# alenzhao/Mitty

Hardware: AMD Instinct MI355X
Metric: paired 2x150bp reads/sec at 30x WGS, 1/2/4/8 MI355X; qname POS/CIGAR bit-exact (higher is better)
Workload: dtype int64+u8

## Files before the change

### include/mitty_hip.h

```cpp
#ifndef MITTY_HIP_H
#define MITTY_HIP_H

#include <stdint.h>

#ifdef __cplusplus
extern "C" {
#endif

typedef struct mh_ctx mh_ctx;

enum {
  MH_OK = 0,
  MH_E_ARG = -1,
  MH_E_HIP = -2,
  MH_E_OOM = -3,
  MH_E_CAPACITY = -4,
  MH_E_COMPLEX_VARIANT = -5,
  MH_E_SEED = -6,
  MH_E_STATE = -7,
  MH_E_NO_DEVICE = -8
};

enum { MH_RNG_MITTY = 0, MH_RNG_PHILOX = 1 };

int32_t mh_version(void);
int32_t mh_device_count(int32_t *out);
int32_t mh_create(int32_t device, mh_ctx **out);
int32_t mh_destroy(mh_ctx *ctx);
const char *mh_last_error(const mh_ctx *ctx);
int32_t mh_sync(mh_ctx *ctx);

int32_t mh_selftest_scan_fault(mh_ctx *ctx);
int32_t mh_selftest_scan(mh_ctx *ctx, int32_t kind, int32_t fields, const int64_t *in, int64_t n, int32_t repeat,
                         int64_t *incl, int64_t *excl, int64_t *total, int64_t *info);
int32_t mh_selftest_sort(mh_ctx *ctx, const uint32_t *keys, int64_t n, int32_t end_bit, uint32_t *keys_out,
                         uint32_t *vals_out);

int32_t mh_read_model_params(int64_t mean_rlen, double coverage, double *p, int64_t *passes);
int32_t mh_work_units(uint64_t seed, const int32_t *ploidy, int64_t n_regions, int64_t passes,
                      int32_t *out_region, int32_t *out_cpy, uint32_t *out_seed, int64_t *out_n);

int32_t mh_upload_contig(mh_ctx *ctx, int32_t contig_id, const char *seq, int64_t len);
int32_t mh_release_contig(mh_ctx *ctx, int32_t contig_id);
int32_t mh_build_haplotype(mh_ctx *ctx, int32_t slot, int32_t contig_id, int64_t ref_start_pos,
                           const int64_t *v_pos, const uint8_t *v_op, const int64_t *v_oplen,
                           const int64_t *v_alt_off, const int64_t *v_alt_len, const char *alt_pool,
                           int64_t alt_pool_len, int64_t n_var,
                           int64_t *out_n_nodes, int64_t *out_p_min, int64_t *out_p_max);
int32_t mh_upload_variants(mh_ctx *ctx, int32_t vset, const int64_t *v_pos, const uint8_t *v_op,
                           const int64_t *v_oplen, const int64_t *v_alt_off, const int64_t *v_alt_len,
                           const char *alt_pool, int64_t alt_pool_len, int64_t n_var);
int32_t mh_build_haplotype_vset(mh_ctx *ctx, int32_t slot, int32_t contig_id, int64_t ref_start_pos, int32_t vset,
                                int64_t *out_n_nodes, int64_t *out_p_min, int64_t *out_p_max);
int32_t mh_build_haplotypes_vset(mh_ctx *ctx, int32_t n, const int32_t *slots, const int32_t *contig_ids,
                                 const int64_t *ref_starts, const int32_t *vsets, int64_t *out_n_nodes,
                                 int64_t *out_p_min, int64_t *out_p_max);
int32_t mh_prefetch_haplotypes_vset(mh_ctx *ctx, int32_t n, const int32_t *slots, const int32_t *contig_ids,
                                    const int64_t *ref_starts, const int32_t *vsets, int32_t n_units,
                                    const int32_t *unit_slots, const uint64_t *unit_seeds, double p);
int32_t mh_release_variants(mh_ctx *ctx, int32_t vset);
int32_t mh_get_nodes(mh_ctx *ctx, int32_t slot, int64_t *ps, int64_t *pr, uint8_t *op, int64_t *oplen,
                     char *hap, int64_t hap_cap, int64_t *hap_len);
int32_t mh_get_haplotype_aux(mh_ctx *ctx, int32_t slot, char *rc, int64_t rc_cap, int64_t *hap_len,
                             int64_t *run_start, int64_t *run_end, int64_t run_cap, int64_t *n_runs,
                             int32_t *bkt, int64_t bkt_cap, int64_t *n_bkt);
int32_t mh_release_haplotype(mh_ctx *ctx, int32_t slot);
int32_t mh_expand_variant(int64_t samp_pos, int64_t ref_pos, int64_t ref_start_pos, int64_t v_pos, int32_t op,
                          int64_t oplen, int64_t *out, int32_t *n_nodes, int64_t *samp_next, int64_t *ref_next);

int32_t mh_sample_templates(mh_ctx *ctx, int32_t slot, double p, int32_t rlen, const double *cum_tlen,
                            int32_t n_tlen, uint64_t seed, int32_t rng_mode, int64_t *out_n_templates);
int32_t mh_sample_templates_span(mh_ctx *ctx, int64_t p_min, int64_t p_max, double p, int32_t rlen,
                                 const double *cum_tlen, int32_t n_tlen, uint64_t seed, int32_t rng_mode,
                                 int64_t *out_n_templates);
int32_t mh_sample_units(mh_ctx *ctx, int32_t n_units, const int32_t *tpl_ids, const int32_t *slots,
                        const uint64_t *seeds, double p, int32_t rlen, const double *cum_tlen, int32_t n_tlen,
                        int32_t rng_mode, int64_t *out_n);
int32_t mh_sample_units_async(mh_ctx *ctx, int32_t n_units, const int32_t *tpl_ids, const int32_t *slots,
                              const uint64_t *seeds, double p, int32_t rlen, const double *cum_tlen, int32_t n_tlen,
                              int32_t rng_mode);
int32_t mh_templates_count(mh_ctx *ctx, int32_t tpl_id, int64_t *n);
int32_t mh_use_templates(mh_ctx *ctx, int32_t tpl_id);
int32_t mh_release_templates(mh_ctx *ctx, int32_t tpl_id);
int32_t mh_set_templates(mh_ctx *ctx, const int8_t *fo0, const int64_t *pos0, const int64_t *pos1, int64_t n,
                         int32_t rlen);
int32_t mh_get_templates(mh_ctx *ctx, int8_t *fo0, int64_t *pos0, int64_t *pos1, int64_t cap, int64_t *n);
int32_t mh_templates_export(mh_ctx *ctx, int32_t tpl_id, int32_t on_device, int8_t *fo0, int64_t *pos0,
                            int64_t *pos1, int64_t cap, int64_t *n);
int32_t mh_templates_import(mh_ctx *ctx, int32_t tpl_id, int32_t on_device, const int8_t *fo0, const int64_t *pos0,
                            const int64_t *pos1, int64_t n, int32_t rlen);
#define MH_GC_BINS 101
int32_t mh_gc_thin(mh_ctx *ctx, int32_t tpl_id, int32_t slot, const uint64_t *accept , uint64_t seed,
                   uint64_t unit_key, int64_t *out_n, int64_t *bin_seen ,
                   int64_t *bin_kept );

int32_t mh_emit_reads(mh_ctx *ctx, int32_t slot, const char *serial_stub, const char *chrom, int64_t cpy,
                      int32_t write_fastq2, uint64_t unit_key, int64_t *out_kept, int64_t *out_bytes1,
                      int64_t *out_bytes2);
int32_t mh_emit_prepare(mh_ctx *ctx, int32_t slot, const char *serial_stub, const char *chrom, int64_t cpy,
                        int32_t write_fastq2, uint64_t unit_key, int64_t *out_kept, int64_t *out_b1, int64_t *out_b2);
int32_t mh_emit_reads_range(mh_ctx *ctx, int32_t slot, const char *serial_stub, const char *chrom, int64_t cpy,
                            int32_t write_fastq2, uint64_t unit_key, int64_t t_begin, int64_t t_end,
                            int64_t cnt_base, int64_t *out_kept, int64_t *out_bytes1, int64_t *out_bytes2);
int32_t mh_emit_reads_async(mh_ctx *ctx, int32_t slot, const char *serial_stub, const char *chrom, int64_t cpy,
                            int32_t write_fastq2, uint64_t unit_key);
int32_t mh_emit_collect(mh_ctx *ctx, int64_t *out, int64_t cap, int64_t *n_units);
int32_t mh_emit_measure(mh_ctx *ctx, int32_t slot, const char *serial_stub, const char *chrom, int64_t cpy,
                        int32_t write_fastq2, uint64_t unit_key, int64_t t_begin, int64_t t_end, int64_t cnt_base,
                        int64_t *out_kept, int64_t *out_b1, int64_t *out_b2);
int32_t mh_count_kept(mh_ctx *ctx, int32_t slot, int64_t t_begin, int64_t t_end, int64_t *out_kept);
int32_t mh_output_size(mh_ctx *ctx, int64_t *bytes1, int64_t *bytes2);
int32_t mh_output_fetch(mh_ctx *ctx, int64_t offset1, char *fq1, int64_t len1, int64_t offset2, char *fq2,
                        int64_t len2);
int32_t mh_output_fetch_async(mh_ctx *ctx, int64_t offset1, char *fq1, int64_t len1, int64_t offset2, char *fq2,
                              int64_t len2, int32_t *ticket);
int32_t mh_output_fetch_wait(mh_ctx *ctx, int32_t ticket);
int32_t mh_output_reset(mh_ctx *ctx);
int32_t mh_host_alloc(int64_t bytes, void **out);
int32_t mh_host_free(void *p);
// ... 52 lines not shown
int32_t mh_score_add_store(mh_ctx *ctx);
int32_t mh_score_result(mh_ctx *ctx, uint64_t *mq_mat, uint64_t *derr_mat, int64_t *counts);
int32_t mh_score_reset(mh_ctx *ctx);

#define MH_MODEL_NO_RLEN INT64_MAX
int32_t mh_model_begin(mh_ctx *ctx, int32_t n_refs, int32_t every, int32_t min_mq, int32_t max_bq, int32_t max_bp,
                       int32_t max_tlen);
int32_t mh_model_add_records(mh_ctx *ctx, const uint8_t *recs, int64_t len, const int64_t *roff, int64_t n);
int32_t mh_model_add_store(mh_ctx *ctx);
int32_t mh_model_result(mh_ctx *ctx, uint64_t *bq_mat, uint64_t *tlen_mat, int64_t *counts);
int32_t mh_model_reset(mh_ctx *ctx);

#define MH_COV_NO_POS INT64_MAX
int32_t mh_cov_begin(mh_ctx *ctx, int32_t n_refs, const int64_t *lengths, int64_t block_len);
int32_t mh_cov_add_records(mh_ctx *ctx, const uint8_t *recs, int64_t len, const int64_t *roff, int64_t n);
int32_t mh_cov_add_store(mh_ctx *ctx);
int32_t mh_cov_gc(mh_ctx *ctx, int32_t ref_index, int32_t contig_id);
int32_t mh_cov_result(mh_ctx *ctx, int32_t ref_index, uint32_t *n_n, uint32_t *n_gc, int64_t *covered,
                      uint64_t *span_sum, int64_t *min_pos, int64_t *max_end, int64_t n_blocks, int64_t *counts);
int32_t mh_cov_reset(mh_ctx *ctx);

#define MH_BQ_MAX_BP 500
#define MH_BQ_MAX_BQ 100
int32_t mh_bq_begin(mh_ctx *ctx, int32_t n_refs);
int32_t mh_bq_add_records(mh_ctx *ctx, const uint8_t *recs, int64_t len, const int64_t *roff, int64_t n);
int32_t mh_bq_add_store(mh_ctx *ctx);
int32_t mh_bq_result(mh_ctx *ctx, int32_t ref_index, uint64_t *mat, int64_t *counts);
int32_t mh_bq_reset(mh_ctx *ctx);

typedef struct mh_vcf mh_vcf;
int32_t mh_vcf_open(const char *path, const char *sample, mh_vcf **out);
const char *mh_vcf_error(const mh_vcf *v);
int32_t mh_vcf_close(mh_vcf *v);
int32_t mh_vcf_region(mh_vcf *v, const char *chrom, int64_t start0, int64_t end, int32_t *ploidy, int64_t *n_var,
                      int64_t *alt_bytes, int32_t cap);
int32_t mh_vcf_copy(mh_vcf *v, int32_t cpy, int64_t *pos, uint8_t *op, int64_t *oplen, int64_t *alt_off,
                    int64_t *alt_len, char *alt_pool);
int32_t mh_vcf_filter(const char *in_path, const char *sample, int32_t n_regions, const char *chroms,
                      const int64_t *start0, const int64_t *end, const char *out_path, int32_t bgzf, int32_t threads,
                      int64_t *n_written, int64_t *n_filtered, char *err, int32_t err_cap);

typedef struct mh_fasta mh_fasta;
int32_t mh_fasta_open(const char *path, const char *names, mh_fasta **out);
const char *mh_fasta_error(const mh_fasta *f);
int32_t mh_fasta_count(const mh_fasta *f, int32_t *n);
int32_t mh_fasta_contig(const mh_fasta *f, int32_t i, const char **name, const char **seq, int64_t *len);
int32_t mh_fasta_copy(const mh_fasta *f, int32_t i, char *dst);
int32_t mh_fasta_close(mh_fasta *f);

int32_t mh_bgzf_compress(const char *in, int64_t len, int32_t level, int32_t threads, char *out, int64_t cap,
                         int64_t *used);
int32_t mh_bgzf_eof(char *out28);
int32_t mh_bgzf_compress_device(mh_ctx *ctx, const void *d_in, int64_t len, void *d_out, int64_t cap,
                                int64_t *used);
int32_t mh_bgzf_compress_gpu(mh_ctx *ctx, const char *in, int64_t len, char *out, int64_t cap, int64_t *used);
int32_t mh_bgzf_inflate_gpu(int32_t device, const char *in, int64_t len, char *out, int64_t cap, int64_t *used,
                            int64_t *bad_offset);
int32_t mh_output_bgzf(mh_ctx *ctx, int32_t file, char *out, int64_t cap, int64_t *used);
int32_t mh_selftest_bgzf(mh_ctx *ctx, const char *in, int64_t len, int32_t misalign, char *out, int64_t cap,
                         int64_t *used);
int32_t mh_output_bgzf_range(mh_ctx *ctx, int32_t file, int64_t offset, int64_t len, char *out, int64_t cap,
                             int64_t *used);
int32_t mh_output_bgzf_pair(mh_ctx *ctx, int64_t offset, int64_t n1, int64_t n2, char *out1, int64_t cap1,
                            char *out2, int64_t cap2, int64_t *used1, int64_t *used2, int32_t *ticket);
int32_t mh_output_bgzf_wait(mh_ctx *ctx, int32_t ticket);

int32_t mh_corrupt_fastq(mh_ctx *ctx, const char *fq1, int64_t len1, const char *fq2, int64_t len2, int64_t t_base,
                         int64_t *used1, int64_t *used2, int64_t *templates);

int32_t mh_set_corruption(mh_ctx *ctx, int32_t enable, const double *cum_bq, int32_t max_bp, int32_t n_bq,
                          const double *phred_p, uint64_t seed);
int32_t mh_set_corruption_stream(mh_ctx *ctx, int32_t rng_mode, uint64_t seed, const uint32_t *key624, int32_t pos);
int32_t mh_get_corruption_stream(mh_ctx *ctx, uint32_t *key624, int32_t *pos, int64_t *words);

int32_t mh_stage_times(mh_ctx *ctx, const char **names, double *ms, int32_t cap, int32_t *n);
int32_t mh_enable_timing(mh_ctx *ctx, int32_t on);

int32_t mh_mt_window_at(uint32_t seed, uint64_t offset, uint32_t *out624);
int32_t mh_set_emit_mode(mh_ctx *ctx, int32_t mode);
#define MH_DEC_SEQUENTIAL 1
#define MH_DEC_FORCE_FIXUP 2
#define MH_DEC_FORCE_GEO 4
int32_t mh_set_decode_mode(mh_ctx *ctx, int32_t mode);
int32_t mh_fixup_count(mh_ctx *ctx, int64_t *n);

#ifdef __cplusplus
}
#endif
#endif
```

### mitty_amd/_native.py

```python
import ctypes
import os
import sys

import numpy as np

LIB_PATH = (os.environ.get('MH_LIB') or
            os.path.join(os.path.dirname(os.path.abspath(__file__)), '_lib', 'libmitty_hip.so'))

MH_OK, MH_E_ARG, MH_E_HIP, MH_E_OOM, MH_E_CAPACITY, MH_E_COMPLEX_VARIANT, MH_E_SEED, MH_E_STATE, MH_E_NO_DEVICE = \
  0, -1, -2, -3, -4, -5, -6, -7, -8
MH_RNG_MITTY, MH_RNG_PHILOX = 0, 1

EXPORTS = ['mh_version', 'mh_device_count', 'mh_create', 'mh_destroy', 'mh_last_error', 'mh_sync',
           'mh_selftest_scan_fault', 'mh_selftest_scan', 'mh_selftest_sort', 'mh_selftest_bgzf',
           'mh_read_model_params', 'mh_work_units', 'mh_upload_contig', 'mh_release_contig', 'mh_build_haplotype', 'mh_upload_variants', 'mh_build_haplotype_vset', 'mh_build_haplotypes_vset', 'mh_prefetch_haplotypes_vset', 'mh_release_variants', 'mh_get_nodes', 'mh_get_haplotype_aux',
           'mh_release_haplotype', 'mh_expand_variant', 'mh_sample_templates', 'mh_sample_templates_span', 'mh_set_templates',
           'mh_get_templates', 'mh_templates_export', 'mh_templates_import', 'mh_gc_thin', 'mh_emit_reads', 'mh_emit_prepare', 'mh_emit_reads_async', 'mh_emit_collect', 'mh_output_size', 'mh_output_fetch', 'mh_output_reset', 'mh_host_alloc', 'mh_host_free', 'mh_device_cache_trim', 'mh_device_live_bytes',
           'mh_read_batch', 'mh_set_corruption', 'mh_set_corruption_stream', 'mh_get_corruption_stream', 'mh_stage_times', 'mh_enable_timing', 'mh_sample_units', 'mh_sample_units_async', 'mh_templates_count',
           'mh_use_templates', 'mh_release_templates', 'mh_mt_window_at', 'mh_fixup_count', 'mh_set_emit_mode', 'mh_set_decode_mode',
           'mh_emit_reads_range', 'mh_emit_measure', 'mh_count_kept', 'mh_bam_set_refs', 'mh_bam_add_fastq', 'mh_bam_add_output',
           'mh_bam_records', 'mh_bam_set_capacity', 'mh_bam_set_spill_dir', 'mh_bam_spilled', 'mh_bam_export', 'mh_bam_import', 'mh_bam_sort', 'mh_bam_write', 'mh_bam_write_gpu', 'mh_bam_reset', 'mh_bam_partition', 'mh_bam_partition_fetch', 'mh_bam_import_tie', 'mh_bam_sorted_head', 'mh_bam_write_part', 'mh_bam_bai_runs', 'mh_corrupt_fastq', 'mh_bgzf_compress', 'mh_bgzf_eof', 'mh_bgzf_compress_device', 'mh_bgzf_compress_gpu', 'mh_output_bgzf',
           'mh_output_bgzf_range', 'mh_output_bgzf_pair', 'mh_output_bgzf_wait', 'mh_output_fetch_async',
           'mh_output_fetch_wait',
           'mh_vcf_open', 'mh_vcf_error', 'mh_vcf_close', 'mh_vcf_region', 'mh_vcf_copy', 'mh_vcf_filter',
           'mh_bamfile_open', 'mh_bamfile_open_gpu', 'mh_bgzf_inflate_gpu', 'mh_bamfile_error', 'mh_bamfile_header', 'mh_bamfile_next', 'mh_bamfile_close',
           'mh_score_begin', 'mh_score_add_records', 'mh_score_add_store', 'mh_score_result', 'mh_score_reset',
           'mh_model_begin', 'mh_model_add_records', 'mh_model_add_store', 'mh_model_result', 'mh_model_reset',
           'mh_cov_begin', 'mh_cov_add_records', 'mh_cov_add_store', 'mh_cov_gc', 'mh_cov_result', 'mh_cov_reset',
           'mh_bq_begin', 'mh_bq_add_records', 'mh_bq_add_store', 'mh_bq_result', 'mh_bq_reset',
           'mh_fasta_open', 'mh_fasta_error', 'mh_fasta_count', 'mh_fasta_contig', 'mh_fasta_copy', 'mh_fasta_close']


MODEL_NO_RLEN = (1 << 63) - 1
GC_BINS = 101
MASK64 = (1 << 64) - 1
COV_NO_POS = (1 << 63) - 1
BQ_MAX_BP, BQ_MAX_BQ = 500, 100


class NativeError(RuntimeError):
  pass


class NativeUnavailable(NativeError):
  pass


_lib = None

c_i32, c_i64, c_u64, c_dbl, c_vp = ctypes.c_int32, ctypes.c_int64, ctypes.c_uint64, ctypes.c_double, ctypes.c_void_p
P_i64 = ctypes.POINTER(c_i64)


def _sig(L, name, args, res=c_i32):
  f = getattr(L, name)
  f.argtypes = args
  f.restype = res


def lib():
  global _lib
  if _lib is not None:
    return _lib
  if not os.path.exists(LIB_PATH):
    raise NativeUnavailable('libmitty_hip.so not built ({}); run __graft_entry__.build() or make -C '
                            'mitty_amd/csrc'.format(LIB_PATH))
  if 'torch' not in sys.modules and int(os.environ.get('WORLD_SIZE', '1')) > 1:
    import torch
  L = ctypes.CDLL(LIB_PATH)
  _sig(L, 'mh_version', [])
  _sig(L, 'mh_device_count', [ctypes.POINTER(c_i32)])
  _sig(L, 'mh_create', [c_i32, ctypes.POINTER(c_vp)])
  _sig(L, 'mh_destroy', [c_vp])
  _sig(L, 'mh_last_error', [c_vp], ctypes.c_char_p)
  _sig(L, 'mh_sync', [c_vp])
  _sig(L, 'mh_selftest_scan_fault', [c_vp])
  _sig(L, 'mh_selftest_scan', [c_vp, c_i32, c_i32, c_vp, c_i64, c_i32, c_vp, c_vp, c_vp, c_vp])
  _sig(L, 'mh_selftest_sort', [c_vp, c_vp, c_i64, c_i32, c_vp, c_vp])
  _sig(L, 'mh_selftest_bgzf', [c_vp, c_vp, c_i64, c_i32, c_vp, c_i64, P_i64])
  _sig(L, 'mh_read_model_params', [c_i64, c_dbl, ctypes.POINTER(c_dbl), P_i64])
  _sig(L, 'mh_work_units', [c_u64, c_vp, c_i64, c_i64, c_vp, c_vp, c_vp, P_i64])
  _sig(L, 'mh_upload_contig', [c_vp, c_i32, c_vp, c_i64])
  _sig(L, 'mh_release_contig', [c_vp, c_i32])
  _sig(L, 'mh_upload_variants', [c_vp, c_i32, c_vp, c_vp, c_vp, c_vp, c_vp, c_vp, c_i64, c_i64])
  _sig(L, 'mh_build_haplotype_vset', [c_vp, c_i32, c_i32, c_i64, c_i32, c_vp, c_vp, c_vp])
  _sig(L, 'mh_release_variants', [c_vp, c_i32])
  _sig(L, 'mh_build_haplotype', [c_vp, c_i32, c_i32, c_i64, c_vp, c_vp, c_vp, c_vp, c_vp, c_vp, c_i64, c_i64,
                                 P_i64, P_i64, P_i64])
  _sig(L, 'mh_get_nodes', [c_vp, c_i32, c_vp, c_vp, c_vp, c_vp, c_vp, c_i64, P_i64])
  _sig(L, 'mh_get_haplotype_aux', [c_vp, c_i32, c_vp, c_i64, P_i64, c_vp, c_vp, c_i64, P_i64, c_vp, c_i64, P_i64])
  _sig(L, 'mh_release_haplotype', [c_vp, c_i32])
  _sig(L, 'mh_bgzf_compress_device', [c_vp, c_vp, c_i64, c_vp, c_i64, P_i64])
  _sig(L, 'mh_bgzf_compress_gpu', [c_vp, c_vp, c_i64, c_vp, c_i64, P_i64])
  _sig(L, 'mh_output_bgzf', [c_vp, c_i32, c_vp, c_i64, P_i64])
  _sig(L, 'mh_output_bgzf_range', [c_vp, c_i32, c_i64, c_i64, c_vp, c_i64, P_i64])
  _sig(L, 'mh_output_bgzf_pair', [c_vp, c_i64, c_i64, c_i64, c_vp, c_i64, c_vp, c_i64, P_i64, P_i64,
                                  ctypes.POINTER(c_i32)])
  _sig(L, 'mh_output_bgzf_wait', [c_vp, c_i32])
  _sig(L, 'mh_output_fetch_async', [c_vp, c_i64, c_vp, c_i64, c_i64, c_vp, c_i64, ctypes.POINTER(c_i32)])
  _sig(L, 'mh_output_fetch_wait', [c_vp, c_i32])
  _sig(L, 'mh_expand_variant', [c_i64, c_i64, c_i64, c_i64, c_i32, c_i64, P_i64, ctypes.POINTER(c_i32), P_i64, P_i64])
  _sig(L, 'mh_sample_templates', [c_vp, c_i32, c_dbl, c_i32, c_vp, c_i32, c_u64, c_i32, P_i64])
  _sig(L, 'mh_sample_templates_span', [c_vp, c_i64, c_i64, c_dbl, c_i32, c_vp, c_i32, c_u64, c_i32, P_i64])
  _sig(L, 'mh_set_templates', [c_vp, c_vp, c_vp, c_vp, c_i64, c_i32])
  _sig(L, 'mh_get_templates', [c_vp, c_vp, c_vp, c_vp, c_i64, P_i64])
  _sig(L, 'mh_emit_reads', [c_vp, c_i32, ctypes.c_char_p, ctypes.c_char_p, c_i64, c_i32, c_u64, P_i64, P_i64, P_i64])
  _sig(L, 'mh_emit_prepare', [c_vp, c_i32, ctypes.c_char_p, ctypes.c_char_p, c_i64, c_i32, c_u64, P_i64, P_i64, P_i64])
  _sig(L, 'mh_emit_reads_async', [c_vp, c_i32, ctypes.c_char_p, ctypes.c_char_p, c_i64, c_i32, c_u64])
  _sig(L, 'mh_emit_collect', [c_vp, c_vp, c_i64, P_i64])
  _sig(L, 'mh_build_haplotypes_vset', [c_vp, c_i32, c_vp, c_vp, c_vp, c_vp, c_vp, c_vp, c_vp])
  _sig(L, 'mh_prefetch_haplotypes_vset', [c_vp, c_i32, c_vp, c_vp, c_vp, c_vp, c_i32, c_vp, c_vp, c_dbl])
  _sig(L, 'mh_emit_reads_range', [c_vp, c_i32, ctypes.c_char_p, ctypes.c_char_p, c_i64, c_i32, c_u64, c_i64, c_i64,
                                   c_i64, P_i64, P_i64, P_i64])
  _sig(L, 'mh_count_kept', [c_vp, c_i32, c_i64, c_i64, P_i64])
  _sig(L, 'mh_emit_measure', [c_vp, c_i32, ctypes.c_char_p, ctypes.c_char_p, c_i64, c_i32, c_u64, c_i64, c_i64, c_i64,
                              P_i64, P_i64, P_i64])
  _sig(L, 'mh_bam_set_refs', [c_vp, c_i32, ctypes.c_char_p, c_vp])
  _sig(L, 'mh_bam_add_fastq', [c_vp, c_vp, c_i64, c_vp, c_i64, c_i64, P_i64, P_i64, P_i64])
  _sig(L, 'mh_bam_add_output', [c_vp, c_i64, P_i64])
  _sig(L, 'mh_bam_records', [c_vp, P_i64, P_i64])
  _sig(L, 'mh_bam_set_capacity', [c_vp, c_i64])
  _sig(L, 'mh_bam_spilled', [c_vp, P_i64, P_i64])
  _sig(L, 'mh_bam_export', [c_vp, c_i64, c_i64, c_vp, c_vp, c_vp, c_vp])
  _sig(L, 'mh_bam_import', [c_vp, c_vp, c_vp, c_vp, c_vp, c_i64])
  _sig(L, 'mh_bam_partition', [c_vp, c_vp, c_i32, ctypes.c_uint64, c_vp, c_vp, c_vp])
  _sig(L, 'mh_bam_set_spill_dir', [c_vp, ctypes.c_char_p])
  _sig(L, 'mh_bam_partition_fetch', [c_vp, c_vp, c_i64])
  _sig(L, 'mh_bam_import_tie', [c_vp, c_vp, c_vp, c_vp, c_vp, c_vp, c_i64])
  _sig(L, 'mh_bam_sorted_head', [c_vp, c_i64, c_vp])
  _sig(L, 'mh_bam_write_part', [c_vp, ctypes.c_char_p, ctypes.c_char_p, c_i64, c_i64, c_vp, c_i64, c_i32, P_i64,
                                P_i64, P_i64, c_vp, c_i64])
  _sig(L, 'mh_bam_bai_runs', [c_vp, P_i64, c_vp, c_i64, P_i64, c_vp, c_i64, c_vp])
  _sig(L, 'mh_bam_write', [c_vp, ctypes.c_char_p, ctypes.c_char_p, c_i64, c_i32, c_i32, ctypes.c_char_p, P_i64,
                           P_i64])
  _sig(L, 'mh_bam_write_gpu', [c_vp, ctypes.c_char_p, ctypes.c_char_p, c_i64, ctypes.c_char_p, P_i64, P_i64, P_i64])
  _sig(L, 'mh_bam_reset', [c_vp])
  _sig(L, 'mh_bam_sort', [c_vp])
  _sig(L, 'mh_corrupt_fastq', [c_vp, c_vp, c_i64, c_vp, c_i64, c_i64, P_i64, P_i64, P_i64])
  _sig(L, 'mh_bgzf_compress', [c_vp, c_i64, c_i32, c_i32, c_vp, c_i64, P_i64])
  _sig(L, 'mh_bgzf_eof', [c_vp])
  _sig(L, 'mh_vcf_open', [ctypes.c_char_p, ctypes.c_char_p, ctypes.POINTER(c_vp)])
  _sig(L, 'mh_vcf_error', [c_vp], ctypes.c_char_p)
  _sig(L, 'mh_vcf_close', [c_vp])
  _sig(L, 'mh_vcf_region', [c_vp, ctypes.c_char_p, c_i64, c_i64, ctypes.POINTER(c_i32), c_vp, c_vp, c_i32])
  _sig(L, 'mh_vcf_copy', [c_vp, c_i32, c_vp, c_vp, c_vp, c_vp, c_vp, c_vp])
  _sig(L, 'mh_vcf_filter', [ctypes.c_char_p, ctypes.c_char_p, c_i32, c_vp, c_vp, c_vp, ctypes.c_char_p, c_i32, c_i32,
                            P_i64, P_i64, ctypes.c_char_p, c_i32])
  _sig(L, 'mh_bamfile_open', [ctypes.c_char_p, c_i32, ctypes.POINTER(c_vp)])
  _sig(L, 'mh_bamfile_open_gpu', [ctypes.c_char_p, c_i32, c_i32, ctypes.POINTER(c_vp)])
  _sig(L, 'mh_bgzf_inflate_gpu', [c_i32, c_vp, c_i64, c_vp, c_i64, P_i64, P_i64])
  _sig(L, 'mh_bamfile_error', [c_vp], ctypes.c_char_p)
  _sig(L, 'mh_bamfile_header', [c_vp, ctypes.POINTER(c_vp), P_i64, ctypes.POINTER(c_i32), ctypes.POINTER(c_vp),
                                ctypes.POINTER(c_vp)])
  _sig(L, 'mh_bamfile_next', [c_vp, c_i64, ctypes.POINTER(c_vp), P_i64, ctypes.POINTER(c_vp), P_i64])
  _sig(L, 'mh_bamfile_close', [c_vp])
  _sig(L, 'mh_score_begin', [c_vp, c_i32, ctypes.c_char_p, c_i32, c_i32, c_i32, ctypes.c_char_p])
  _sig(L, 'mh_score_add_records', [c_vp, c_vp, c_i64, c_vp, c_i64])
  _sig(L, 'mh_score_add_store', [c_vp])
  _sig(L, 'mh_score_result', [c_vp, c_vp, c_vp, c_vp])
  _sig(L, 'mh_score_reset', [c_vp])
  _sig(L, 'mh_model_begin', [c_vp, c_i32, c_i32, c_i32, c_i32, c_i32, c_i32])
  _sig(L, 'mh_model_add_records', [c_vp, c_vp, c_i64, c_vp, c_i64])
  _sig(L, 'mh_model_add_store', [c_vp])
  _sig(L, 'mh_model_result', [c_vp, c_vp, c_vp, c_vp])
  _sig(L, 'mh_model_reset', [c_vp])
  _sig(L, 'mh_cov_begin', [c_vp, c_i32, c_vp, c_i64])
  _sig(L, 'mh_cov_add_records', [c_vp, c_vp, c_i64, c_vp, c_i64])
  _sig(L, 'mh_cov_add_store', [c_vp])
  _sig(L, 'mh_cov_gc', [c_vp, c_i32, c_i32])
  _sig(L, 'mh_cov_result', [c_vp, c_i32, c_vp, c_vp, c_vp, c_vp, c_vp, c_vp, c_i64, c_vp])
  _sig(L, 'mh_cov_reset', [c_vp])
  _sig(L, 'mh_bq_begin', [c_vp, c_i32])
  _sig(L, 'mh_bq_add_records', [c_vp, c_vp, c_i64, c_vp, c_i64])
  _sig(L, 'mh_bq_add_store', [c_vp])
  _sig(L, 'mh_bq_result', [c_vp, c_i32, c_vp, c_vp])
  _sig(L, 'mh_bq_reset', [c_vp])
  _sig(L, 'mh_fasta_open', [ctypes.c_char_p, c_vp, ctypes.POINTER(c_vp)])
  _sig(L, 'mh_fasta_error', [c_vp], ctypes.c_char_p)
  _sig(L, 'mh_fasta_count', [c_vp, ctypes.POINTER(c_i32)])
  _sig(L, 'mh_fasta_contig', [c_vp, c_i32, ctypes.POINTER(ctypes.c_char_p), ctypes.POINTER(c_vp), P_i64])
  _sig(L, 'mh_fasta_copy', [c_vp, c_i32, c_vp])
  _sig(L, 'mh_fasta_close', [c_vp])
  _sig(L, 'mh_output_size', [c_vp, P_i64, P_i64])
  _sig(L, 'mh_output_fetch', [c_vp, c_i64, c_vp, c_i64, c_i64, c_vp, c_i64])
  _sig(L, 'mh_output_reset', [c_vp])
  _sig(L, 'mh_host_alloc', [c_i64, ctypes.POINTER(c_vp)])
  _sig(L, 'mh_host_free', [c_vp])
  _sig(L, 'mh_device_cache_trim', [ctypes.POINTER(c_i64)])
  _sig(L, 'mh_device_live_bytes', [ctypes.POINTER(c_i64), ctypes.POINTER(c_i64), c_i32])
  _sig(L, 'mh_read_batch', [c_vp, c_i32, c_vp, c_vp, c_i64, c_vp, c_vp, c_vp,
                            c_vp, c_i64, c_vp, P_i64, c_vp, c_i64, c_vp, P_i64, c_vp, c_i64, c_vp, P_i64])
  _sig(L, 'mh_set_corruption', [c_vp, c_i32, c_vp, c_i32, c_i32, c_vp, c_u64])
  _sig(L, 'mh_templates_export', [c_vp, c_i32, c_i32, c_vp, c_vp, c_vp, c_i64, P_i64])
  _sig(L, 'mh_templates_import', [c_vp, c_i32, c_i32, c_vp, c_vp, c_vp, c_i64, c_i32])
  _sig(L, 'mh_gc_thin', [c_vp, c_i32, c_i32, c_vp, c_u64, c_u64, P_i64, c_vp, c_vp])
  _sig(L, 'mh_set_corruption_stream', [c_vp, c_i32, c_u64, c_vp, c_i32])
  _sig(L, 'mh_get_corruption_stream', [c_vp, c_vp, ctypes.POINTER(c_i32), P_i64])
  _sig(L, 'mh_stage_times', [c_vp, ctypes.POINTER(ctypes.c_char_p), ctypes.POINTER(c_dbl), c_i32,
                             ctypes.POINTER(c_i32)])
  _sig(L, 'mh_enable_timing', [c_vp, c_i32])
  _sig(L, 'mh_sample_units', [c_vp, c_i32, c_vp, c_vp, c_vp, c_dbl, c_i32, c_vp, c_i32, c_i32, c_vp])
  _sig(L, 'mh_sample_units_async', [c_vp, c_i32, c_vp, c_vp, c_vp, c_dbl, c_i32, c_vp, c_i32, c_i32])
  _sig(L, 'mh_templates_count', [c_vp, c_i32, c_vp])
  _sig(L, 'mh_use_templates', [c_vp, c_i32])
  _sig(L, 'mh_release_templates', [c_vp, c_i32])
  _sig(L, 'mh_mt_window_at', [ctypes.c_uint32, c_u64, c_vp])
  _sig(L, 'mh_fixup_count', [c_vp, P_i64])
  _sig(L, 'mh_set_emit_mode', [c_vp, c_i32])
  _sig(L, 'mh_set_decode_mode', [c_vp, c_i32])
  _lib = L
  return L


def mt_window_at(seed, offset):
  out = np.empty(624, np.uint32)
  rc = lib().mh_mt_window_at(int(seed), int(offset), _ptr(out))
  if rc:
    _raise(rc, 'mh_mt_window_at failed')
  return out


def bgzf_compress(data, level=6, threads=8):
  n = len(data)
  src = np.frombuffer(data, np.uint8) if n else np.zeros(1, np.uint8)
  cap = n + (n // 0xff00 + 1) * 64 + 64
  out = np.empty(cap, np.uint8)
  used = c_i64()
  rc = lib().mh_bgzf_compress(_ptr(src), n, int(level), int(threads), _ptr(out), cap, ctypes.byref(used))
  if rc == MH_E_CAPACITY:
    out = np.empty(used.value, np.uint8)
    rc = lib().mh_bgzf_compress(_ptr(src), n, int(level), int(threads), _ptr(out), used.value, ctypes.byref(used))
  if rc:
    _raise(rc, 'mh_bgzf_compress failed')
  return out[:used.value].tobytes()


class VcfFile:

  def __init__(self, path, sample):
    L = lib()
    self._L = L
    self._h = c_vp()
    rc = L.mh_vcf_open(path.encode(), sample.encode(), ctypes.byref(self._h))
    if rc:
      msg = L.mh_vcf_error(self._h).decode() if self._h else 'mh_vcf_open failed'
      self.close()
      _raise(rc, msg)

  def close(self):
    if getattr(self, '_h', None):
      self._L.mh_vcf_close(self._h)
      self._h = None

  def __del__(self):
    try:
      self.close()
    except Exception:
      pass

  def region(self, chrom, start0, end):
    pl = c_i32()
    nv = np.zeros(64, np.int64)
    ab = np.zeros(64, np.int64)
    rc = self._L.mh_vcf_region(self._h, chrom.encode(), int(start0), int(end), ctypes.byref(pl), _ptr(nv), _ptr(ab),
                               64)
    if rc:
      _raise(rc, self._L.mh_vcf_error(self._h).decode())
    copies = []
    for c in range(pl.value):
      n, nb = int(nv[c]), int(ab[c])
      pos, oplen, aoff, alen = (np.empty(n, np.int64) for _ in range(4))
      op = np.empty(n, np.uint8)
      pool = np.empty(max(nb, 1), np.uint8)
      rc = self._L.mh_vcf_copy(self._h, c, _ptr(pos), _ptr(op), _ptr(oplen), _ptr(aoff), _ptr(alen), _ptr(pool))
      if rc:
        _raise(rc, self._L.mh_vcf_error(self._h).decode())
      copies.append({'pos': pos, 'op': op, 'oplen': oplen, 'alt_off': aoff, 'alt_len': alen,
                     'alt_pool': pool[:nb].tobytes()})
    return pl.value, copies


class BamFile:

  def __init__(self, path, threads=2, device=None):
    L = lib()
    self._L = L
    self._h = c_vp()
    if device is None:
      rc = L.mh_bamfile_open(path.encode(), int(threads), ctypes.byref(self._h))
    else:
      rc = L.mh_bamfile_open_gpu(path.encode(), int(device), int(threads), ctypes.byref(self._h))
    if rc:
# ... 294 lines not shown
    us, ud = a(unit_slots, np.int32), a(unit_seeds, np.uint64)
    self._chk(self._L.mh_prefetch_haplotypes_vset(self._h, n, _ptr(s), _ptr(c), _ptr(r), _ptr(v), nu, _ptr(us),
                                                  _ptr(ud), float(p)))

  def release_variants(self, vset):
    self._chk(self._L.mh_release_variants(self._h, int(vset)))

  def get_nodes(self, slot, n_nodes, with_hap=True):
    ps, pr, ol = (np.empty(max(n_nodes, 1), np.int64) for _ in range(3))
    op = np.empty(max(n_nodes, 1), np.uint8)
    hl = c_i64()
    self._chk(self._L.mh_get_nodes(self._h, slot, None, None, None, None, None, 0, ctypes.byref(hl)))
    hap = np.empty(max(hl.value, 1), np.uint8) if with_hap else None
    self._chk(self._L.mh_get_nodes(self._h, slot, _ptr(ps), _ptr(pr), _ptr(op), _ptr(ol), _ptr(hap),
                                   hl.value if with_hap else 0, ctypes.byref(hl)))
    return ps[:n_nodes], pr[:n_nodes], op[:n_nodes], ol[:n_nodes], (hap[:hl.value].tobytes() if with_hap else None)

  def get_haplotype_aux(self, slot):
    hl, nr, nb = c_i64(), c_i64(), c_i64()
    self._chk(self._L.mh_get_haplotype_aux(self._h, slot, None, 0, ctypes.byref(hl), None, None, 0, ctypes.byref(nr),
                                           None, 0, ctypes.byref(nb)))
    rc = np.empty(max(hl.value, 1), np.uint8)
    rs, re_ = np.empty(max(nr.value, 1), np.int64), np.empty(max(nr.value, 1), np.int64)
    bkt = np.empty(nb.value + 1, np.int32)
    self._chk(self._L.mh_get_haplotype_aux(self._h, slot, _ptr(rc), hl.value, ctypes.byref(hl), _ptr(rs), _ptr(re_),
                                           nr.value, ctypes.byref(nr), _ptr(bkt), nb.value + 1, ctypes.byref(nb)))
    return rc[:hl.value].tobytes(), rs[:nr.value], re_[:nr.value], bkt

  def release_haplotype(self, slot):
    self._chk(self._L.mh_release_haplotype(self._h, slot))

  def sample_templates(self, slot, p, rlen, cum_tlen, seed, rng_mode=MH_RNG_MITTY):
    ct = np.ascontiguousarray(cum_tlen, dtype=np.float64)
    n = c_i64()
    self._chk(self._L.mh_sample_templates(self._h, slot, float(p), int(rlen), _ptr(ct), len(ct), int(seed),
                                          int(rng_mode), ctypes.byref(n)))
    return n.value

  def sample_templates_span(self, p_min, p_max, p, rlen, cum_tlen, seed, rng_mode=MH_RNG_MITTY):
    if not (0 <= int(seed) <= 0xffffffff):
      raise ValueError('Seed value {} is out of range 0 - {}'.format(seed, 0xffffffff))
    ct = np.ascontiguousarray(cum_tlen, dtype=np.float64)
    n = c_i64()
    self._chk(self._L.mh_sample_templates_span(self._h, int(p_min), int(p_max), float(p), int(rlen), _ptr(ct),
                                               len(ct), int(seed), int(rng_mode), ctypes.byref(n)))
    return n.value

  def sample_units(self, tpl_ids, slots, seeds, p, rlen, cum_tlen, rng_mode=MH_RNG_MITTY):
    ids = np.ascontiguousarray(tpl_ids, dtype=np.int32)
    sl = np.ascontiguousarray(slots, dtype=np.int32)
    sd = np.ascontiguousarray(seeds, dtype=np.uint64)
    ct = np.ascontiguousarray(cum_tlen, dtype=np.float64)
    out = np.zeros(max(len(ids), 1), dtype=np.int64)
    self._chk(self._L.mh_sample_units(self._h, len(ids), _ptr(ids), _ptr(sl), _ptr(sd), float(p), int(rlen),
                                      _ptr(ct), len(ct), int(rng_mode), _ptr(out)))
    return out[:len(ids)]

  def sample_units_async(self, tpl_ids, slots, seeds, p, rlen, cum_tlen, rng_mode=MH_RNG_MITTY):
    ids = np.ascontiguousarray(tpl_ids, dtype=np.int32)
    sl = np.ascontiguousarray(slots, dtype=np.int32)
    sd = np.ascontiguousarray(seeds, dtype=np.uint64)
    ct = np.ascontiguousarray(cum_tlen, dtype=np.float64)
    self._chk(self._L.mh_sample_units_async(self._h, len(ids), _ptr(ids), _ptr(sl), _ptr(sd), float(p), int(rlen),
                                            _ptr(ct), len(ct), int(rng_mode)))
    return len(ids)

  def template_count(self, tpl_id):
    n = c_i64()
    self._chk(self._L.mh_templates_count(self._h, int(tpl_id), ctypes.byref(n)))
    return n.value

  def use_templates(self, tpl_id):
    self._chk(self._L.mh_use_templates(self._h, int(tpl_id)))

  def release_templates(self, tpl_id):
    self._chk(self._L.mh_release_templates(self._h, int(tpl_id)))

  def set_emit_mode(self, mode):
    self._chk(self._L.mh_set_emit_mode(self._h, int(mode)))

  def set_decode_mode(self, mode):
    self._chk(self._L.mh_set_decode_mode(self._h, int(mode)))

  def fixup_count(self):
    n = c_i64()
    self._chk(self._L.mh_fixup_count(self._h, ctypes.byref(n)))
    return n.value

  def set_templates(self, fo0, pos0, pos1, rlen):
    fo0 = np.ascontiguousarray(fo0, dtype=np.int8)
    pos0 = np.ascontiguousarray(pos0, dtype=np.int64)
    pos1 = np.ascontiguousarray(pos1, dtype=np.int64)
    self._chk(self._L.mh_set_templates(self._h, _ptr(fo0), _ptr(pos0), _ptr(pos1), len(fo0), int(rlen)))

  def get_templates(self):
    n = c_i64()
    self._L.mh_get_templates(self._h, None, None, None, 0, ctypes.byref(n))
    m = n.value
    fo0, p0, p1 = np.empty(max(m, 1), np.int8), np.empty(max(m, 1), np.int64), np.empty(max(m, 1), np.int64)
    self._chk(self._L.mh_get_templates(self._h, _ptr(fo0), _ptr(p0), _ptr(p1), max(m, 1), ctypes.byref(n)))
    return fo0[:m], p0[:m], p1[:m]

  def emit_prepare(self, slot, serial_stub, chrom, cpy, write_fastq2=True, unit_key=0, wait=True):
    if not wait:
      self._chk(self._L.mh_emit_prepare(self._h, slot, serial_stub.encode(), chrom.encode(), int(cpy),
                                        1 if write_fastq2 else 0, int(unit_key), None, None, None))
      return None
    k, b1, b2 = c_i64(), c_i64(), c_i64()
    self._chk(self._L.mh_emit_prepare(self._h, slot, serial_stub.encode(), chrom.encode(), int(cpy),
                                      1 if write_fastq2 else 0, int(unit_key), ctypes.byref(k), ctypes.byref(b1),
                                      ctypes.byref(b2)))
    return k.value, b1.value, b2.value

  def emit_reads(self, slot, serial_stub, chrom, cpy, write_fastq2=True, unit_key=0, t_range=None, cnt_base=0):
    k, b1, b2 = c_i64(), c_i64(), c_i64()
    if t_range is None:
      self._chk(self._L.mh_emit_reads(self._h, slot, serial_stub.encode(), chrom.encode(), int(cpy),
                                      1 if write_fastq2 else 0, int(unit_key), ctypes.byref(k), ctypes.byref(b1),
                                      ctypes.byref(b2)))
    else:
      self._chk(self._L.mh_emit_reads_range(self._h, slot, serial_stub.encode(), chrom.encode(), int(cpy),
                                            1 if write_fastq2 else 0, int(unit_key), int(t_range[0]),
                                            int(t_range[1]), int(cnt_base), ctypes.byref(k), ctypes.byref(b1),
                                            ctypes.byref(b2)))
    return k.value, b1.value, b2.value

  def emit_async(self, slot, serial_stub, chrom, cpy, write_fastq2=True, unit_key=0):
    self._chk(self._L.mh_emit_reads_async(self._h, slot, serial_stub.encode(), chrom.encode(), int(cpy),
                                          1 if write_fastq2 else 0, int(unit_key)))

  def emit_collect(self):
    n = c_i64()
    self._chk(self._L.mh_emit_collect(self._h, None, 0, ctypes.byref(n)))
    out = np.zeros(3 * max(n.value, 1), np.int64)
    self._chk(self._L.mh_emit_collect(self._h, _ptr(out), n.value, ctypes.byref(n)))
    return [tuple(int(x) for x in out[3 * i:3 * i + 3]) for i in range(n.value)]

  def emit_measure(self, slot, serial_stub, chrom, cpy, write_fastq2=True, unit_key=0, t_range=None, cnt_base=0):
    k, b1, b2 = c_i64(), c_i64(), c_i64()
    t0, t1 = t_range if t_range is not None else (0, -1)
    self._chk(self._L.mh_emit_measure(self._h, slot, serial_stub.encode(), chrom.encode(), int(cpy),
                                      1 if write_fastq2 else 0, int(unit_key), int(t0), int(t1), int(cnt_base),
                                      ctypes.byref(k), ctypes.byref(b1), ctypes.byref(b2)))
    return k.value, b1.value, (b2.value if write_fastq2 else 0)

  def bgzf_range(self, f, off, n, pin):
    if n <= 0:
      return b''
    cap = n + (n // 0xff00 + 2) * 40 + 64
    pin.reserve(cap)
    used = c_i64()
    self._chk(self._L.mh_output_bgzf_range(self._h, int(f), int(off), int(n), c_vp(pin.ptr), cap, ctypes.byref(used)))
    return bytes(pin.view(used.value))

  def count_kept(self, slot, t_begin, t_end):
    k = c_i64()
    self._chk(self._L.mh_count_kept(self._h, slot, int(t_begin), int(t_end), ctypes.byref(k)))
    return k.value

  def output_size(self):
    a, b = c_i64(), c_i64()
    self._chk(self._L.mh_output_size(self._h, ctypes.byref(a), ctypes.byref(b)))
    return a.value, b.value

  def fetch_output(self, off1=0, len1=None, off2=0, len2=None):
    u1, u2 = self.output_size()
# ... 355 lines not shown
    caps = [max(64, 64 * n), max(64, 16 * n), max(64, int(l.sum()) + 16 if n else 64)]
    for _ in range(2):
      bufs = [np.empty(c, np.uint8) for c in caps]
      rc = self._L.mh_read_batch(self._h, slot, _ptr(p), _ptr(l), n, _ptr(pos), _ptr(n0), _ptr(n1),
                                 _ptr(bufs[0]), caps[0], _ptr(offs[0]), ctypes.byref(used[0]),
                                 _ptr(bufs[1]), caps[1], _ptr(offs[1]), ctypes.byref(used[1]),
                                 _ptr(bufs[2]), caps[2], _ptr(offs[2]), ctypes.byref(used[2]))
      if rc == MH_E_CAPACITY:
        caps = [max(c, u.value + 16) for c, u in zip(caps, used)]
        continue
      self._chk(rc)
      break
    texts = [b[:u.value].tobytes().decode('latin-1') for b, u in zip(bufs, used)]
    return pos[:n], n0[:n], n1[:n], texts, offs

  def set_corruption(self, enable, cum_bq=None, phred_p=None, seed=0):
    if not enable:
      self._chk(self._L.mh_set_corruption(self._h, 0, None, 0, 0, None, 0))
      return
    cb = np.ascontiguousarray(cum_bq, dtype=np.float64)
    ph = np.ascontiguousarray(phred_p, dtype=np.float64)
    self._chk(self._L.mh_set_corruption(self._h, 1, _ptr(cb), cb.shape[1], cb.shape[2], _ptr(ph), int(seed)))

  def templates_export(self, tpl_id, fo0=None, pos0=None, pos1=None, cap=None):
    n = c_i64()
    if fo0 is not None:
      self._chk(self._L.mh_templates_export(self._h, int(tpl_id), 1, c_vp(fo0), c_vp(pos0), c_vp(pos1), int(cap),
                                            ctypes.byref(n)))
      return n.value
    self._L.mh_templates_export(self._h, int(tpl_id), 0, None, None, None, 0, ctypes.byref(n))
    m = n.value
    a, b, c = np.empty(max(m, 1), np.int8), np.empty(max(m, 1), np.int64), np.empty(max(m, 1), np.int64)
    self._chk(self._L.mh_templates_export(self._h, int(tpl_id), 0, _ptr(a), _ptr(b), _ptr(c), max(m, 1),
                                          ctypes.byref(n)))
    return a[:m], b[:m], c[:m]

  def templates_import(self, tpl_id, n, rlen, fo0, pos0, pos1, on_device=False):
    if on_device:
      self._chk(self._L.mh_templates_import(self._h, int(tpl_id), 1, c_vp(fo0), c_vp(pos0), c_vp(pos1), int(n),
                                            int(rlen)))
      return
    a = np.ascontiguousarray(fo0, dtype=np.int8)
    b = np.ascontiguousarray(pos0, dtype=np.int64)
    c = np.ascontiguousarray(pos1, dtype=np.int64)
    self._chk(self._L.mh_templates_import(self._h, int(tpl_id), 0, _ptr(a), _ptr(b), _ptr(c), int(n), int(rlen)))

  def gc_thin(self, tpl_id, slot, accept, seed, unit_key):
    acc = np.ascontiguousarray(accept, dtype=np.uint64)
    if acc.shape != (GC_BINS,):
      raise ValueError('gc_thin: {} thresholds needed, got an array of shape {}'.format(GC_BINS, acc.shape))
    n = c_i64()
    seen, kept = np.zeros(GC_BINS, np.int64), np.zeros(GC_BINS, np.int64)
    self._chk(self._L.mh_gc_thin(self._h, int(tpl_id), int(slot), _ptr(acc), int(seed) & MASK64, int(unit_key) & MASK64,
                                 ctypes.byref(n), _ptr(seen), _ptr(kept)))
    return n.value, seen, kept

  def set_corruption_stream(self, rng_mode, seed=0, key=None, pos=624):
    k = None if key is None else np.ascontiguousarray(key, dtype=np.uint32)
    if k is not None and k.shape != (624,):
      raise ValueError('MT19937 key must hold 624 words')
    self._chk(self._L.mh_set_corruption_stream(self._h, int(rng_mode), int(seed), None if k is None else _ptr(k),
                                               int(pos)))

  def get_corruption_stream(self):
    key = np.empty(624, np.uint32)
    pos, words = c_i32(), c_i64()
    self._chk(self._L.mh_get_corruption_stream(self._h, _ptr(key), ctypes.byref(pos), ctypes.byref(words)))
    return key, pos.value, words.value

  def enable_timing(self, on=True):
    self._chk(self._L.mh_enable_timing(self._h, 1 if on else 0))

  def stage_times(self):
    n = c_i32()
    self._L.mh_stage_times(self._h, None, None, 0, ctypes.byref(n))
    names = (ctypes.c_char_p * max(n.value, 1))()
    ms = (c_dbl * max(n.value, 1))()
    self._L.mh_stage_times(self._h, names, ms, n.value, ctypes.byref(n))
    return [(names[i].decode(), ms[i]) for i in range(n.value)]

  def sync(self):
    self._chk(self._L.mh_sync(self._h))

  def selftest_sort(self, keys, end_bit):
    import numpy as np
    k = np.ascontiguousarray(keys, dtype=np.uint32)
    ko, vo = np.empty_like(k), np.empty_like(k)
    self._chk(self._L.mh_selftest_sort(self._h, k.ctypes.data, k.size, int(end_bit), ko.ctypes.data, vo.ctypes.data))
    return ko, vo

  def selftest_scan(self, kind, x, repeat=1):
    x = np.ascontiguousarray(x, dtype=np.int64)
    if x.ndim not in (1, 2):
      raise ValueError('selftest_scan: a 1-d or 2-d array')
    fields = 1 if x.ndim == 1 else x.shape[1]
    n = x.shape[0]
    scans = int(kind) != 3
    incl = np.empty_like(x) if scans else None
    excl = np.empty_like(x) if scans else None
    total, info = np.zeros(max(fields, 1), np.int64), np.zeros(2, np.int64)
    self._chk(self._L.mh_selftest_scan(self._h, int(kind), int(fields), _ptr(x), n, int(repeat), _ptr(incl),
                                       _ptr(excl), _ptr(total), _ptr(info)))
    return incl, excl, (total[0] if x.ndim == 1 else total), (int(info[0]), int(info[1]))

  def selftest_bgzf(self, data, misalign=0):
    n = len(data)
    if n == 0:
      return b''
    src = np.frombuffer(data, np.uint8)
    out = np.empty(n + (n // 0xff00 + 2) * 40 + 64, np.uint8)
    used = c_i64()
    self._chk(self._L.mh_selftest_bgzf(self._h, _ptr(src), n, int(misalign), _ptr(out), len(out), ctypes.byref(used)))
    return out[:used.value].tobytes()

  def selftest_scan_fault(self):
    rc = self._L.mh_selftest_scan_fault(self._h)
    return rc, self._L.mh_last_error(self._h).decode(errors='replace')


def expand_variant(samp_pos, ref_pos, ref_start_pos, v_pos, op, oplen):
  out = (c_i64 * 10)()
  n, sn, rn = c_i32(), c_i64(), c_i64()
  rc = lib().mh_expand_variant(int(samp_pos), int(ref_pos), int(ref_start_pos), int(v_pos), ord(op), int(oplen), out,
                               ctypes.byref(n), ctypes.byref(sn), ctypes.byref(rn))
  if rc:
    _raise(rc, 'mh_expand_variant: bad variant (op {!r}, oplen {})'.format(op, oplen))
  return [(out[5 * j], out[5 * j + 1], chr(out[5 * j + 2]), out[5 * j + 3], out[5 * j + 4])
          for j in range(n.value)], sn.value, rn.value
```

### mitty_amd/csrc/mh_api.hip

```cpp
#include <sys/mman.h>
#include <sys/syscall.h>
#include <unistd.h>

#include <algorithm>
#include <atomic>
#include <cctype>
#include <cstdio>
#include <unordered_map>
#include <chrono>
#include <cmath>
#include <condition_variable>
#include <cstring>
#include <map>
#include <mutex>
#include <thread>
#include <type_traits>

#include "mh_bgzf.h"
#include <vector>

#include "mh_corrupt.h"
#include "mh_internal.h"
#include "mh_scan.h"
#include "mh_sort.h"
// ... 422 lines not shown
      hipEventCreateWithFlags(&ctx->ev_ready, hipEventDisableTiming) != hipSuccess ||
      hipEventCreateWithFlags(&ctx->ev_writer, hipEventDisableTiming) != hipSuccess ||
      [&] {
        for (auto &e : ctx->eset)
          if (hipEventCreateWithFlags(&e.done, hipEventDisableTiming) != hipSuccess ||
              hipEventCreateWithFlags(&e.rb, hipEventDisableTiming) != hipSuccess ||
              hipHostMalloc((void **)&e.h_stat, 64 + 8192, hipHostMallocDefault) != hipSuccess)
            return true;
        return false;
      }()) {
    delete ctx;
    return MH_E_HIP;
  }
  hipDeviceProp_t prop;
  if (hipGetDeviceProperties(&prop, device) == hipSuccess) ctx->max_cu = prop.multiProcessorCount;
  *out = ctx;
  return MH_OK;
}

int32_t mh_destroy(mh_ctx *ctx) {
  if (!ctx) return MH_OK;
  if (ctx->pf_thread.joinable()) ctx->pf_thread.join();
  (void)hipSetDevice(ctx->device);
  (void)hipStreamSynchronize(ctx->wstream);
  (void)hipStreamSynchronize(ctx->stream);
  if (ctx->stream2) (void)hipStreamSynchronize(ctx->stream2);
  if (ctx->pstream) (void)hipStreamSynchronize(ctx->pstream);
  for (auto x : ctx->xstream)
    if (x) (void)hipStreamSynchronize(x);
  for (auto &kv : ctx->contigs) release(kv.second.seq);
  for (auto &kv : ctx->haps) release_hap(kv.second);
  for (auto &h : ctx->hap_spare) release_hap(h);
  for (auto &kv : ctx->vsets) release_vars(kv.second);
  for (auto &kv : ctx->tsets) {
    release(kv.second.fo0); release(kv.second.pos0); release(kv.second.pos1); release(kv.second.n0);
    if (kv.second.used) (void)hipEventDestroy(kv.second.used);
  }
  release(ctx->jump_polys); release(ctx->perm_tmp); release(ctx->nrun_tmp); release(ctx->dec_buf);
  release(ctx->gc_buf);
  for (auto &b : ctx->gc_out) release(b);
  for (auto &b : ctx->pb) release(b);
  release(ctx->pb_tmp);
  release(ctx->gz_slots); release(ctx->gz_tok); release(ctx->gz_info); release(ctx->gz_off); release(ctx->gz_scan); release(ctx->gz_out);
  release(ctx->gz_in);
  for (auto &b : ctx->s) release(b);
  for (auto &b : ctx->lane2) release(b);
  for (auto &l : ctx->xlane)
    for (auto &b : l) release(b);
  for (auto &b : ctx->xscan) release(b);
  release(ctx->scan_partials); release(ctx->scan_partials2); release(ctx->d_small);
  release(ctx->corrupt_cum); release(ctx->corrupt_phred);
  release(ctx->out1); release(ctx->out2);
  release(ctx->cr_rows);
  release(ctx->cr_codes);
  release(ctx->scan_partials_w);
  for (auto &b : ctx->sl2) release(b);
  for (auto &b : ctx->sl3) release(b);
  ctx->tail_state.reset();
  for (hipEvent_t e : ctx->ev_gz)
    if (e) (void)hipEventDestroy(e);
  for (hipEvent_t e : ctx->ev_fetch)
    if (e) (void)hipEventDestroy(e);
  if (ctx->h_small) (void)hipHostFree(ctx->h_small);
  if (ctx->h_small3) (void)hipHostFree(ctx->h_small3);
  if (ctx->h_units) (void)hipHostFree(ctx->h_units);
  for (uint8_t *p : ctx->h_bam_pin)
    if (p) (void)hipHostFree(p);
  for (auto &e : ctx->eset) {
    release(e.recs); release(e.off); release(e.tsum); release(e.tpre); release(e.stat); release(e.crrec);
    (void)hipEventDestroy(e.done);
    if (e.rb) (void)hipEventDestroy(e.rb);
    if (e.h_stat) (void)hipHostFree(e.h_stat);
  }
  (void)hipEventDestroy(ctx->ev_ready);
  (void)hipEventDestroy(ctx->ev_writer);
  (void)hipStreamDestroy(ctx->wstream);
  bam_release(ctx->bam);
  score_release(ctx->score);
  model_release(ctx->model);
  model_release(ctx->bq);
  cov_release(ctx->cov);
  if (ctx->ev_fork) (void)hipEventDestroy(ctx->ev_fork);
  if (ctx->ev_join) (void)hipEventDestroy(ctx->ev_join);
  if (ctx->stream2) (void)hipStreamDestroy(ctx->stream2);
  if (ctx->ev_prefetch) (void)hipEventDestroy(ctx->ev_prefetch);
  if (ctx->pstream) (void)hipStreamDestroy(ctx->pstream);
  for (int l = 0; l < 2; l++) {
    if (ctx->xstream[l]) (void)hipStreamDestroy(ctx->xstream[l]);
    if (ctx->ev_xjoin[l]) (void)hipEventDestroy(ctx->ev_xjoin[l]);
  }
  (void)hipStreamDestroy(ctx->stream);
  delete ctx;
  return MH_OK;
}

const char *mh_last_error(const mh_ctx *ctx) { return ctx ? ctx->err.c_str() : "null context"; }

int32_t mh_sync(mh_ctx *ctx) {
  CTX_GUARD(ctx);
  MH_TRY(lazy_resolve(ctx));
  SYNCCHK(ctx, hipStreamSynchronize(ctx->stream));
  return MH_OK;
}

namespace {
struct LoadOne {
  __device__ int64_t operator()(int64_t) const { return 1; }
};
struct StoreCheck {
  int32_t *bad;
  __device__ void operator()(int64_t i, int64_t, int64_t ex) const {
    if (ex != i) atomicOr(bad, 1);
  }
};
}

int32_t mh_selftest_sort(mh_ctx *ctx, const uint32_t *keys, int64_t n, int32_t end_bit, uint32_t *keys_out,
                         uint32_t *vals_out) {
  CTX_GUARD(ctx);
  if (n < 0 || (n > 0 && (!keys || !keys_out || !vals_out)) || end_bit < 0 || end_bit > 32)
    return arg_fail(ctx, MH_E_ARG, "bad sort arguments");
  hipStream_t st = ctx->stream;
  size_t tmp = 0;
  HIPCHK(ctx, lsd_sort_pairs_iota(nullptr, tmp, nullptr, nullptr, nullptr, n, (unsigned)end_bit, st));
  DevBuf b;
  const size_t kb = (4 * (size_t)n + 255) & ~(size_t)255;
  MH_TRY(ensure(ctx, b, 3 * kb + tmp + 256));
  uint32_t *dk = (uint32_t *)b.p, *ko = (uint32_t *)((char *)b.p + kb), *vo = (uint32_t *)((char *)b.p + 2 * kb);
  const int32_t rc = [&]() -> int32_t {
    if (n) HIPCHK(ctx, hipMemcpyAsync(dk, keys, 4 * (size_t)n, hipMemcpyHostToDevice, st));
    HIPCHK(ctx, lsd_sort_pairs_iota((char *)b.p + 3 * kb, tmp, dk, ko, vo, n, (unsigned)end_bit, st));
    if (n) {
      HIPCHK(ctx, hipMemcpyAsync(keys_out, ko, 4 * (size_t)n, hipMemcpyDeviceToHost, st));
      HIPCHK(ctx, hipMemcpyAsync(vals_out, vo, 4 * (size_t)n, hipMemcpyDeviceToHost, st));
    }
    SYNCCHK(ctx, hipStreamSynchronize(st));
    return MH_OK;
  }();
  release(b);
  return rc;
}

int32_t mh_selftest_scan(mh_ctx *ctx, int32_t kind, int32_t fields, const int64_t *in, int64_t n, int32_t repeat,
                         int64_t *incl, int64_t *excl, int64_t *total, int64_t *info) {
  CTX_GUARD(ctx);
  if (kind < 0 || kind > 3 || fields < 1 || fields > 3 || (kind == 1 && fields != 1) || n < 0 ||
      n > ((int64_t)1 << 27) || repeat < 1 || repeat > (1 << 20) || ((kind == 1 || kind == 3) && repeat != 1) ||
      !total || !info || (n > 0 && (!in || (kind != 3 && (!incl || !excl)))))
    return arg_fail(ctx, MH_E_ARG, "bad scan self-test arguments");
  if (kind == 2) {
    uint64_t sum[3] = {0, 0, 0};
    for (int64_t i = 0; i < n * fields; i++) {
      if (in[i] < 0) return arg_fail(ctx, MH_E_ARG, "look-back scan: a negative input");
      uint64_t &s = sum[i % fields];
      s += (uint64_t)in[i];
      if (s >= ((uint64_t)1 << 46)) return arg_fail(ctx, MH_E_ARG, "look-back scan: a field's total is 2^46 or more");
    }
  }
  info[0] = info[1] = 0;
  if (fields == 1) return selftest_scan_run<int64_t>(ctx, kind, in, n, repeat, incl, excl, total, info);
  if (fields == 2) return selftest_scan_run<Sc2>(ctx, kind, in, n, repeat, incl, excl, total, info);
  return selftest_scan_run<Sc3>(ctx, kind, in, n, repeat, incl, excl, total, info);
}

int32_t mh_selftest_scan_fault(mh_ctx *ctx) {
  CTX_GUARD(ctx);
  hipStream_t st = ctx->stream;
  const int64_t n = 2 * (int64_t)LB_TILE + 5;
  MH_TRY(ensure(ctx, ctx->scan_partials, scan_lb_scratch_bytes<int64_t>(n)));
  MH_TRY(ensure(ctx, ctx->scan_partials2, scan_lb_scratch_bytes<int64_t>(n)));
  MH_TRY(ensure(ctx, ctx->d_small, 8192 + 256));
  int64_t *tot = (int64_t *)((char *)ctx->d_small.p + 160);
  int32_t *bad = (int32_t *)((char *)ctx->d_small.p + 168);
  auto fault_once = [&](hipStream_t s, void *scratch) -> int32_t {
    HIPCHK(ctx, hipMemsetAsync(bad, 0, 4, s));
    HIPCHK(ctx, device_scan_sum<int64_t>(s, n, LoadOne{}, StoreCheck{bad}, scratch, tot, true));
    SYNCCHK(ctx, hipStreamSynchronize(s));
    return MH_OK;
  };
  int32_t rc_lane = MH_OK;
  std::thread t1([&]() {
    lane_thread_enter(ctx);
    if (hipSetDevice(ctx->device) != hipSuccess) {
      rc_lane = MH_E_HIP;
      return;
    }
    rc_lane = fault_once(ctx->stream2, ctx->scan_partials2.p);
  });
  t1.join();
  if (rc_lane != MH_E_STATE) return arg_fail(ctx, MH_E_HIP, "the timed-out scan of a lane thread was not reported");
  const int32_t rc = fault_once(st, ctx->scan_partials.p);
  if (rc != MH_E_STATE) return arg_fail(ctx, MH_E_HIP, "the timed-out scan was not reported");
  const std::string msg = ctx->err;
  HIPCHK(ctx, hipMemsetAsync(bad, 0, 4, st));
  HIPCHK(ctx, device_scan_sum<int64_t>(st, n, LoadOne{}, StoreCheck{bad}, ctx->scan_partials.p, tot));
  int32_t hb = 0;
  HIPCHK(ctx, hipMemcpyAsync(&hb, bad, 4, hipMemcpyDeviceToHost, st));
  SYNCCHK(ctx, hipStreamSynchronize(st));
  if (hb) return arg_fail(ctx, MH_E_HIP, "the scan after the fault is wrong");
  arg_fail(ctx, MH_E_STATE, msg);
  return MH_E_STATE;
}

int32_t mh_read_model_params(int64_t mean_rlen, double coverage, double *p_out, int64_t *passes_out) {
  if (!p_out || !passes_out || mean_rlen <= 0) return MH_E_ARG;
  double p = 1.0;
  int64_t passes = 1;
  while (p > 0.1) {
    passes *= 2;
    p = 0.5 * coverage / (double)(2 * mean_rlen * passes);
  }
  *p_out = p;
  *passes_out = passes;
  return MH_OK;
// ... 864 lines not shown

int32_t mh_host_alloc(int64_t bytes, void **out) {
  if (!out || bytes < 0) return MH_E_ARG;
  *out = nullptr;
  const size_t n = (size_t)(bytes > 0 ? bytes : 1);
  int dev = 0;
  const int node = hipGetDevice(&dev) == hipSuccess ? mh::gpu_numa_node(dev) : -1;
  if (node >= 0 && node < 1024) {
    void *p = mmap(nullptr, n, PROT_READ | PROT_WRITE, MAP_PRIVATE | MAP_ANONYMOUS, -1, 0);
    if (p != MAP_FAILED) {
      unsigned long mask[1024 / (8 * sizeof(unsigned long))] = {0};
      mask[node / (8 * sizeof(unsigned long))] |= 1ul << (node % (8 * sizeof(unsigned long)));
      const long rc = syscall(SYS_mbind, p, n, 2 , mask, (unsigned long)1024, 0u);
      if (rc == 0 && hipHostRegister(p, n, hipHostRegisterDefault) == hipSuccess) {
        std::lock_guard<std::mutex> lk(mh::host_allocs_mu());
        mh::host_allocs()[p] = n;
        *out = p;
        return MH_OK;
      }
      (void)hipGetLastError();
      munmap(p, n);
    }
  }
  if (hipHostMalloc(out, n, hipHostMallocDefault) != hipSuccess) return MH_E_OOM;
  return MH_OK;
}

int32_t mh_device_cache_trim(int64_t *freed_bytes) {
  const int64_t f = mh::cache_trim(-1);
  if (freed_bytes) *freed_bytes = f;
  return MH_OK;
}

int32_t mh_device_live_bytes(int64_t *live, int64_t *peak, int32_t reset_peak) {
  if (live) *live = mh::g_live.load();
  if (peak) *peak = mh::g_live_peak.load();
  if (reset_peak) mh::g_live_peak.store(mh::g_live.load());
  return MH_OK;
}

int32_t mh_host_free(void *p) {
  if (!p) return MH_OK;
  size_t n = 0;
  {
    std::lock_guard<std::mutex> lk(mh::host_allocs_mu());
    auto it = mh::host_allocs().find(p);
    if (it != mh::host_allocs().end()) {
      n = it->second;
      mh::host_allocs().erase(it);
    }
  }
  if (n) {
    const hipError_t e = hipHostUnregister(p);
    munmap(p, n);
    return e == hipSuccess ? MH_OK : MH_E_HIP;
  }
  if (hipHostFree(p) != hipSuccess) return MH_E_HIP;
  return MH_OK;
}

int32_t mh_mt_window_at(uint32_t seed, uint64_t offset, uint32_t *out624) {
  if (!out624) return MH_E_ARG;
  try {
    mh::jump::window_at(seed, offset, out624);
  } catch (...) {
    return MH_E_ARG;
  }
  return MH_OK;
}

int32_t mh_set_emit_mode(mh_ctx *ctx, int32_t mode) {
  if (!ctx || mode < 0 || mode > 3) return MH_E_ARG;
  ctx->emit_lds_only = mode == 1;
  ctx->emit_two_pass = mode == 2;
  ctx->emit_single = mode == 3;
  return MH_OK;
}

int32_t mh_set_decode_mode(mh_ctx *ctx, int32_t mode) {
  if (!ctx || mode < 0 || mode > (MH_DEC_SEQUENTIAL | MH_DEC_FORCE_FIXUP | MH_DEC_FORCE_GEO)) return MH_E_ARG;
  ctx->decode_sequential = (mode & MH_DEC_SEQUENTIAL) != 0;
  ctx->force_fixup = (mode & MH_DEC_FORCE_FIXUP) != 0;
  ctx->force_geo = (mode & MH_DEC_FORCE_GEO) != 0;
  return MH_OK;
}

int32_t mh_fixup_count(mh_ctx *ctx, int64_t *n) {
  if (!ctx || !n) return MH_E_ARG;
  *n = ctx->fixups;
  return MH_OK;
}

int32_t mh_enable_timing(mh_ctx *ctx, int32_t on) {
  if (!ctx) return MH_E_ARG;
  (void)hipSetDevice(ctx->device);
  stages_collect(ctx);
  ctx->timing = on != 0;
  ctx->last_times.clear();
  return MH_OK;
}

int32_t mh_stage_times(mh_ctx *ctx, const char **names, double *ms, int32_t cap, int32_t *n) {
  if (!ctx || !n) return MH_E_ARG;
  (void)hipSetDevice(ctx->device);
  stages_collect(ctx);
  int32_t k = 0;
  for (auto &t : ctx->last_times) {
    if (k < cap) {
      if (names) names[k] = t.first;
      if (ms) ms[k] = t.second;
    }
    k++;
  }
  *n = k;
  if (names || ms) ctx->last_times.clear();
  return MH_OK;
}

int32_t mh_bam_set_refs(mh_ctx *ctx, int32_t n_refs, const char *names, const int64_t *lengths) {
  CTX_GUARD(ctx);
  if (n_refs < 0 || (n_refs > 0 && (!names || !lengths))) return arg_fail(ctx, MH_E_ARG, "bad reference list");
  return bam_set_refs(ctx, n_refs, names, lengths);
}

static int32_t stage_in(mh_ctx *ctx, DevBuf &b, const char *src, int64_t len) {
  MH_TRY(ensure(ctx, b, (size_t)len + 64));
  if (len) HIPCHK(ctx, hipMemcpyAsync(b.p, src, len, hipMemcpyHostToDevice, ctx->stream));
  HIPCHK(ctx, hipMemsetAsync((char *)b.p + len, 0, 64, ctx->stream));
  return MH_OK;
}

int32_t mh_bam_add_fastq(mh_ctx *ctx, const char *fq1, int64_t len1, const char *fq2, int64_t len2,
                         int64_t max_templates, int64_t *used1, int64_t *used2, int64_t *templates) {
  CTX_GUARD(ctx);
  if (!fq1 || len1 < 0 || (fq2 && len2 < 0) || !used1 || !used2 || !templates)
    return arg_fail(ctx, MH_E_ARG, "null argument");
  MH_TRY(stage_in(ctx, ctx->bam.in1, fq1, len1));
  if (fq2) MH_TRY(stage_in(ctx, ctx->bam.in2, fq2, len2));
  return bam_add(ctx, (const uint8_t *)ctx->bam.in1.p, len1, fq2 ? (const uint8_t *)ctx->bam.in2.p : nullptr,
                 fq2 ? len2 : 0, max_templates, used1, used2, templates);
}

int32_t mh_bam_add_output(mh_ctx *ctx, int64_t max_templates, int64_t *templates) {
  CTX_GUARD(ctx);
  MH_TRY(lazy_resolve(ctx));
  if (!templates) return arg_fail(ctx, MH_E_ARG, "null argument");
  int64_t u1 = 0, u2 = 0;
  const bool two = ctx->used2 > 0;
  const uint8_t *a1 = (const uint8_t *)ctx->out1.p, *a2 = two ? (const uint8_t *)ctx->out2.p : nullptr;
  if (ctx->bam.cap <= 0)
    return bam_add(ctx, a1, ctx->used1, a2, two ? ctx->used2 : 0, max_templates, &u1, &u2, templates, true);
  const int64_t per = std::max<int64_t>(1, ctx->bam.cap / 2048);
  int64_t o1 = 0, o2 = 0, tot = 0;
  int64_t win = per * 4096;
  while (max_templates < 0 || tot < max_templates) {
    const int64_t lim = max_templates < 0 ? per : std::min(per, max_templates - tot);
    const int64_t r1 = ctx->used1 - o1, r2 = two ? ctx->used2 - o2 : 0;
    const int64_t l1 = std::min(r1, win), l2 = std::min(r2, win);
    int64_t t = 0;
    MH_TRY(bam_add(ctx, a1 + o1, l1, two ? a2 + o2 : nullptr, l2, lim, &u1, &u2, &t, false));
    if (t == 0 && (l1 < r1 || l2 < r2)) {
      win *= 2;
      continue;
    }
    if (t == 0) break;
    o1 += u1;
// ... 777 lines not shown
```

### mitty_amd/csrc/mh_internal.h

```cpp
#pragma once

#include <hip/hip_runtime.h>

#include <cstdint>
#include <functional>
#include <map>
#include <mutex>
#include <unordered_map>
#include <memory>
#include <string>
#include <thread>
#include <vector>

#include "../../include/mitty_hip.h"

namespace mh {

struct Status {
  int32_t code = MH_OK;
  std::string msg;
};

#define MH_TRY(expr)                        \
  do {                                      \
// ... 179 lines not shown
  static constexpr int N_REF = 24;
  RecSession ses;
  explicit ModelState(const RecTexts &t) : ses(t) {}
  int32_t n_refs = 0, every = 1, min_mq = 0, max_bq = 0, max_bp = 0, max_tlen = 0;
  int32_t n_tab = 2;
  bool by_ref = false;
  int32_t slab_bp = 0, n_slab = 0;
  int64_t n_bq = 0, n_all = 0;
  DevBuf acc, delta;
  DevBuf desc;
  DevBuf tile_ord;
};

struct CovState {
  static constexpr int N_REF = ModelState::N_REF;
  RecSession ses{COV_TEXTS};
  int32_t n_refs = 0, n_vis = 0;
  int64_t block_len = 0;
  int64_t ln[N_REF] = {0}, cbase[N_REF + 1] = {0}, bbase[N_REF + 1] = {0};
  int64_t n_cells = 0, n_blk = 0;
  DevBuf track, depth;
  DevBuf blk;
  DevBuf cnt;
  DevBuf desc;
  DevBuf partials;
  DevBuf tab;
  bool scanned = false;
};

struct StageTime {
  const char *name;
  hipEvent_t a, b;
};

}

namespace mh {
struct EmitSet {
  DevBuf recs, off;
  DevBuf tsum, tpre;
  DevBuf crrec;
  DevBuf stat;
  int64_t *h_stat = nullptr;
  hipEvent_t rb = nullptr;
  hipEvent_t done = nullptr;
  bool busy = false;
  bool prepared = false;
};
}

struct mh_ctx {
  int fault_slot = 0;
  int device = 0;
  hipStream_t stream = nullptr;
  hipStream_t stream2 = nullptr;
  hipEvent_t ev_fork = nullptr, ev_join = nullptr;
  hipStream_t wstream = nullptr;
  std::shared_ptr<void> tail_state;
  int64_t *h_units = nullptr, *d_units = nullptr;
  hipEvent_t ev_ready = nullptr, ev_writer = nullptr;
  bool writer_pending = false;
  static constexpr int N_ESET = 16;
  mh::EmitSet eset[N_ESET];
  int64_t eset_max_m = 0;
  int eset_i = 0;
  hipStream_t stage_stream = nullptr;
  std::string err;
  int32_t max_cu = 256;

  std::map<int32_t, mh::Contig> contigs;
  std::map<int32_t, mh::Hap> haps;

  std::map<int32_t, mh::TplSet> tsets;
  int32_t cur_tpl = -1;

  mh::DevBuf jump_polys;
  int64_t jump_k = 0, jump_seg = 0;
  int64_t fixups = 0;
  std::map<int32_t, mh::VarSet> vsets;
  std::vector<mh::Hap> hap_spare;
  mh::DevBuf perm_tmp;
  mh::DevBuf pb[6];
  mh::DevBuf pb_tmp;
  mh::DevBuf gz_slots, gz_info, gz_off, gz_scan, gz_out, gz_in;
  mh::DevBuf gz_tok;
  hipEvent_t ev_gz[2] = {nullptr, nullptr};
  hipEvent_t ev_fetch[2] = {nullptr, nullptr};
  bool fetch_pending[2] = {false, false};
  int fetch_next = 0;
  bool gz_pending[2] = {false, false};
  int gz_half = 0;
  mh::DevBuf nrun_tmp;
  mh::DevBuf dec_buf;
  int64_t dec_passes = 0;

  mh::DevBuf s[16];
  mh::DevBuf scan_partials;
  mh::DevBuf lane2[8];
  mh::DevBuf scan_partials2;
  hipStream_t xstream[2] = {nullptr, nullptr};
  mh::DevBuf xlane[2][8];
  mh::DevBuf xscan[2];
  hipEvent_t ev_xjoin[2] = {nullptr, nullptr};
  mh::DevBuf sl2[8];
  hipStream_t pstream = nullptr;
  hipEvent_t ev_prefetch = nullptr;
  bool prefetch_pending = false;
  std::thread pf_thread;
  int32_t pf_rc = 0;
  mh::DevBuf sl3[8];
  int64_t *h_small3 = nullptr;
  mh::PrefetchedWords pf_words;
  mh::DevBuf pinned_small;
  mh::DevBuf d_small;

  bool corrupt_on = false;
  mh::DevBuf corrupt_cum, corrupt_phred;
  int32_t corrupt_max_bp = 0, corrupt_n_bq = 0;
  size_t corrupt_guide_off = 0;
  size_t corrupt_bk_off = 0, corrupt_T16_off = 0, corrupt_Fp16_off = 0;
  size_t corrupt_bkf_off = 0;
  uint64_t corrupt_seed = 0;
  int32_t cx_mode = 0;
  uint32_t cx_seed = 0;
  int64_t cx_pos = 0;
  uint32_t cx_key[624] = {0};
  int32_t cx_kpos = 624;
  mh::DevBuf cx_words, cx_bits, cx_start, cx_aux;

  bool emit_lds_only = false;
  bool decode_sequential = false;
  bool force_fixup = false;
  bool force_geo = false;

  mh::DevBuf out1, out2;
  int64_t used1 = 0, used2 = 0;
  static constexpr int LZ_SLOTS = 4096;
  int64_t *h_lazy = nullptr, *d_lazy = nullptr;
  mh::DevBuf d_cur;
  mh::DevBuf fused_lb;
  struct LazyUnit {
    int32_t slot;
    int64_t gen;
    int64_t known[3];
  };
  std::vector<LazyUnit> lazy;
  std::vector<int64_t> lazy_done;
  int64_t lazy_seq = 0;
  int64_t lazy_gen = 0;
  bool chain_open = false;
  int64_t used_ub1 = 0, used_ub2 = 0;
  int64_t batch_left = 0;
  bool emit_two_pass = false;
  bool emit_single = false;
  mh::DevBuf cr_rows, cr_codes;
  mh::DevBuf scan_partials_w;
  int64_t *h_small = nullptr;
  uint8_t *h_bam_pin[2] = {nullptr, nullptr};

  bool timing = false;
  std::vector<mh::StageTime> stages;
  std::vector<mh::StageTime> pending;
  std::vector<std::pair<const char *, double>> last_times;

  mh::BamStore bam;
  mh::ScoreState score;
// ... 3 lines not shown
  mh::DevBuf gc_out[4];
};

namespace mh {

int32_t hip_fail(mh_ctx *ctx, hipError_t e, const char *what, const char *file, int line);
int32_t arg_fail(mh_ctx *ctx, int32_t code, const std::string &msg);

#define HIPCHK(ctx, call)                                                     \
  do {                                                                        \
    hipError_t _e = (call);                                                   \
    if (_e != hipSuccess) return ::mh::hip_fail((ctx), _e, #call, __FILE__, __LINE__); \
  } while (0)

int32_t scan_fault_fail(mh_ctx *ctx);
#define SYNCCHK(ctx, call)                                                    \
  do {                                                                        \
    HIPCHK(ctx, call);                                                        \
    if (::mh::scan_fault_pending(ctx)) return ::mh::scan_fault_fail(ctx);     \
  } while (0)
bool scan_fault_pending(const mh_ctx *ctx);

int32_t ensure(mh_ctx *ctx, DevBuf &b, size_t bytes);
int32_t ensure_keep(mh_ctx *ctx, DevBuf &b, size_t bytes, size_t keep, int32_t grow_shift = 1);
void release(DevBuf &b);
void release_hap(Hap &h);
int32_t join_writer(mh_ctx *ctx);
int32_t mark_used(mh_ctx *ctx, hipEvent_t &ev, bool &set);
int32_t wait_unused(mh_ctx *ctx, hipEvent_t ev, bool set, hipStream_t st = nullptr);
int32_t join_prefetch(mh_ctx *ctx);
int32_t prefetch_words(mh_ctx *ctx, hipStream_t st, int32_t n_units, const int64_t *p_min, const int64_t *p_max,
                       const uint64_t *seeds, double p);

void stage_begin(mh_ctx *ctx, const char *name);
void stage_end(mh_ctx *ctx);
void stages_collect(mh_ctx *ctx);
struct StageScope {
  mh_ctx *ctx;
  bool open = true;
  StageScope(mh_ctx *c, const char *name) : ctx(c) { stage_begin(c, name); }
  StageScope(const StageScope &) = delete;
  StageScope &operator=(const StageScope &) = delete;
  void end() {
    if (open) stage_end(ctx);
    open = false;
  }
  ~StageScope() { end(); }
};
struct StageStreamScope {
  mh_ctx *ctx;
  hipStream_t prev;
  StageStreamScope(mh_ctx *c, hipStream_t st) : ctx(c), prev(c->stage_stream) { c->stage_stream = st; }
  StageStreamScope(const StageStreamScope &) = delete;
  StageStreamScope &operator=(const StageStreamScope &) = delete;
  ~StageStreamScope() { ctx->stage_stream = prev; }
};

inline void prep_drop(mh_ctx *ctx, const TplSet &tp) {
  if (tp.prep.valid) ctx->eset[tp.prep.set].prepared = false;
  tp.prep.valid = false;
}

inline unsigned grid_for(int64_t n, int threads, int64_t cap = 1 << 20) {
  int64_t g = (n + threads - 1) / threads;
  if (g < 1) g = 1;
  if (g > cap) g = cap;
  return (unsigned)g;
}

int32_t var_upload(mh_ctx *ctx, VarSet &v, const int64_t *v_pos, const uint8_t *v_op, const int64_t *v_oplen,
                   const int64_t *v_alt_off, const int64_t *v_alt_len, const char *alt_pool, int64_t alt_pool_len,
                   int64_t n_var);
void release_vars(VarSet &v);
int32_t splice_build(mh_ctx *ctx, Hap &h, const Contig &c, int64_t ref_start_pos, const VarSet &v, int lane = 0);

int32_t sample_units(mh_ctx *ctx, int32_t n_units, const int32_t *tpl_ids, const int64_t *p_min, const int64_t *p_max,
                     const uint64_t *seeds, double p, int32_t rlen, const double *cum_tlen, int32_t n_tlen,
                     int32_t rng_mode, int64_t *out_n, const NodeIdx *nidx = nullptr);
int32_t sample_units_async(mh_ctx *ctx, int32_t n_units, const int32_t *tpl_ids, const int64_t *p_min,
                           const int64_t *p_max, const uint64_t *seeds, double p, int32_t rlen, const double *cum_tlen,
                           int32_t n_tlen, int32_t rng_mode, const NodeIdx *nidx = nullptr);
int32_t tpl_resolve(mh_ctx *ctx, TplSet &ts);
int32_t tpl_resolve_all(mh_ctx *ctx);

int32_t sync_writers(mh_ctx *ctx);
int32_t bgzf_device(mh_ctx *ctx, hipStream_t st, const uint8_t *d_in, int64_t n, uint8_t *d_out, int64_t cap,
                    int64_t *used, std::vector<int64_t> *boff = nullptr,
                    const std::function<void(int64_t, int64_t)> *on_piece = nullptr);
int64_t bgzf_device_bound(int64_t n);
int gpu_numa_node(int dev);
std::mutex &host_allocs_mu();
std::unordered_map<void *, size_t> &host_allocs();
int64_t *pinned_small(mh_ctx *ctx);
int32_t emit_reads(mh_ctx *ctx, const Hap &h, int32_t slot, const char *serial_stub, const char *chrom, int64_t cpy,
                   int32_t write_fastq2, uint64_t unit_key, int64_t t_begin, int64_t t_end, int64_t cnt_base,
                   bool prepare_only, int64_t *out_kept, int64_t *out_b1, int64_t *out_b2);
int32_t count_kept(mh_ctx *ctx, const Hap &h, int64_t t_begin, int64_t t_end, int64_t *out_kept);
int32_t emit_unit_async(mh_ctx *ctx, const Hap &h, const char *serial_stub, const char *chrom, int64_t cpy,
                        int32_t write_fastq2, uint64_t unit_key, bool *queued);
int32_t lazy_resolve(mh_ctx *ctx);

int32_t bam_set_refs(mh_ctx *ctx, int32_t n_refs, const char *names, const int64_t *lengths);
int32_t bam_add(mh_ctx *ctx, const uint8_t *d1, int64_t len1, const uint8_t *d2, int64_t len2, int64_t max_templates,
                int64_t *used1, int64_t *used2, int64_t *templates, bool sorted_direct = false);
int32_t bam_sort(mh_ctx *ctx, const void *pa = nullptr);
int32_t bam_undirect(mh_ctx *ctx);
int32_t bam_fetch_sorted(mh_ctx *ctx, uint8_t *recs, int64_t *soff, int32_t *info);
int32_t bam_spill(mh_ctx *ctx);
int32_t bam_export(mh_ctx *ctx, int64_t r0, int64_t r1, uint8_t *recs, int64_t *roff, uint64_t *key, int32_t *info);
int32_t bam_import(mh_ctx *ctx, const uint8_t *recs, const int64_t *roff, const uint64_t *key, const int32_t *info,
                   int64_t n, const uint64_t *tie = nullptr);
int32_t bam_partition(mh_ctx *ctx, const uint64_t *split, int32_t n_dest, uint64_t tie_base, int64_t *seg_off,
                      int64_t *seg_n, int64_t *seg_bytes);
int32_t bam_bai_raw(mh_ctx *ctx, std::vector<int64_t> &runs, std::vector<int64_t> &win, std::vector<uint32_t> &nwin,
                    std::vector<int64_t> &woff, bool *ok);
struct BamHostOrder {
  std::vector<uint32_t> val;
  std::vector<int64_t> roff, soff;
};
int32_t bam_host_order(mh_ctx *ctx, BamHostOrder &o);
void bam_assemble(const BamStore &B, const BamHostOrder &o, int64_t w0, int64_t w1, uint8_t *dst, int threads);
struct BaiPlan;
int32_t bam_bai_plan(mh_ctx *ctx, BaiPlan &plan, std::vector<int64_t> &offs, bool *ok);
void bam_release(BamStore &B);
void bam_free_spill(BamStore &B);
int32_t newline_index(mh_ctx *ctx, const uint8_t *b, int64_t len, DevBuf &nl, int64_t *count);
int32_t score_begin(mh_ctx *ctx, int32_t n_refs, const char *names, int32_t max_d, int32_t max_v_len, int32_t strict,
                    const char *sample_prefix);
int32_t score_add_records(mh_ctx *ctx, const uint8_t *recs, int64_t len, const int64_t *roff, int64_t n);
int32_t score_add_store(mh_ctx *ctx);
int32_t score_result(mh_ctx *ctx, uint64_t *mq_mat, uint64_t *derr_mat, int64_t *counts);
int32_t score_reset(mh_ctx *ctx);
void score_release(ScoreState &S);
int32_t model_begin(mh_ctx *ctx, ModelState &S, int32_t n_refs, int32_t every, int32_t min_mq, int32_t max_bq,
                    int32_t max_bp, int32_t max_tlen, bool by_ref);
int32_t model_add_records(mh_ctx *ctx, ModelState &S, const uint8_t *recs, int64_t len, const int64_t *roff,
                          int64_t n);
int32_t model_add_store(mh_ctx *ctx, ModelState &S);
int32_t model_result(mh_ctx *ctx, ModelState &S, uint64_t *bq_mat, uint64_t *tlen_mat, int64_t *counts);
int32_t model_result_table(mh_ctx *ctx, ModelState &S, int32_t tab, uint64_t *mat, int64_t *counts);
int32_t model_reset(mh_ctx *ctx, ModelState &S);
void model_release(ModelState &S);
int32_t cov_begin(mh_ctx *ctx, int32_t n_refs, const int64_t *lengths, int64_t block_len);
int32_t cov_add_records(mh_ctx *ctx, const uint8_t *recs, int64_t len, const int64_t *roff, int64_t n);
int32_t cov_add_store(mh_ctx *ctx);
int32_t cov_gc(mh_ctx *ctx, int32_t ref_index, int32_t contig_id);
int32_t cov_result(mh_ctx *ctx, int32_t ref_index, uint32_t *n_n, uint32_t *n_gc, int64_t *covered, uint64_t *span_sum,
                   int64_t *min_pos, int64_t *max_end, int64_t n_blocks, int64_t *counts);
int32_t cov_reset(mh_ctx *ctx);
void cov_release(CovState &S);
int32_t corrupt_fastq(mh_ctx *ctx, const uint8_t *d0, int64_t len0, const uint8_t *d1, int64_t len1, int64_t t_base,
                      int64_t *used0, int64_t *used1, int64_t *templates);

int32_t read_batch(mh_ctx *ctx, const Hap &h, const int64_t *p, const int64_t *l, int64_t n, int64_t *out_pos,
                   int64_t *out_n0, int64_t *out_n1, char *cigar, int64_t cigar_cap, int64_t *cigar_off,
                   int64_t *cigar_used, char *vlist, int64_t vlist_cap, int64_t *vlist_off, int64_t *vlist_used,
                   char *seq, int64_t seq_cap, int64_t *seq_off, int64_t *seq_used);


int32_t mt_stream_words(mh_ctx *ctx, hipStream_t st, uint32_t seed, int64_t first, int64_t count, DevBuf &out,
                        DevBuf &jobs_buf, int64_t *lead);
int32_t mt_state_words(mh_ctx *ctx, hipStream_t st, const uint32_t *key624, int32_t pos, int64_t count, DevBuf &out,
                       DevBuf &key_buf);

struct CorruptCfg;
CorruptCfg corrupt_cfg(const mh_ctx *ctx, uint64_t unit_key, int64_t t_base);
// ... 12 lines not shown
```

### mitty_amd/csrc/mh_sample.hip

```cpp
#include <algorithm>
#include <cmath>
#include <cstdio>
#include <cstdlib>
#include <cstring>


#include "mh_device.h"
#include "mh_internal.h"
#include "mh_scan.h"
#include "mh_sort.h"


namespace mh {

namespace jump {
void jump_poly_words(uint64_t L, int64_t k, uint32_t *out624);
}

namespace {

constexpr uint32_t MT_UP = 0x80000000u, MT_LO = 0x7fffffffu, MT_A = 0x9908b0dfu;
constexpr int64_t SEG_WORDS_DEFAULT = 624 * 640;
static int64_t seg_words() { return SEG_WORDS_DEFAULT; }

// ... 585 lines not shown

__global__ void __launch_bounds__(SD_THREADS) k_shuffle_decode(uint32_t seed, int64_t n, uint32_t *j) {
  __shared__ uint32_t st[2][624];
  __shared__ uint32_t words[624];
  __shared__ int32_t wave_cnt[SD_WAVES];
  __shared__ int64_t s_i0;
  const int t = threadIdx.x, lane = t & 63, wave = t >> 6;
  if (t == 0) {
    s_i0 = n - 1;
    if (n > 0) j[0] = 0;
  }
  mt_seed_lds(st[0], seed);
  int cur = 0;
  int64_t i0 = n - 1;
  while (i0 >= 1) {
    mt_twist_block(st[cur], st[cur ^ 1], [&](int k, uint32_t w) { words[k] = w; });
    cur ^= 1;
    const bool have = t < 624;
    const uint32_t w = have ? words[t] : 0u;
    int32_t A = t;
    bool acc = false;
    uint32_t v = 0;
    bool converged = false;
    for (int it = 0; it < 16; it++) {
      int64_t i = i0 - A;
      acc = have && i >= 1 && ((v = (w & interval_mask((uint32_t)i))) <= (uint32_t)i);
      uint64_t bal = __ballot(acc);
      if (lane == 0) wave_cnt[wave] = __popcll(bal);
      __syncthreads();
      int32_t pre = 0;
      for (int q = 0; q < wave; q++) pre += wave_cnt[q];
      int32_t A2 = pre + (int32_t)__popcll(bal & ((lane ? (~0ull >> (64 - lane)) : 0ull)));
      int same = __syncthreads_and(A2 == A);
      A = A2;
      if (same) { converged = true; break; }
    }
    if (!converged) {
      if (t == 0) {
        int64_t ii = i0;
        for (int k = 0; k < 624 && ii >= 1; k++) {
          uint32_t vv = words[k] & interval_mask((uint32_t)ii);
          if (vv <= (uint32_t)ii) { j[ii] = vv; ii--; }
        }
        s_i0 = ii;
      }
      __syncthreads();
      i0 = s_i0;
      __syncthreads();
      continue;
    }
    if (acc) j[i0 - A] = v;
    int32_t tot = 0;
    for (int q = 0; q < SD_WAVES; q++) tot += wave_cnt[q];
    i0 -= tot;
    __syncthreads();
  }
}

__global__ void __launch_bounds__(256) k_perm_heads(int64_t n, const uint32_t *K, const uint32_t *V, int32_t *nxt) {
  const int64_t k = (int64_t)blockIdx.x * blockDim.x + threadIdx.x;
  if (k >= n) return;
  const uint32_t b = K[k];
  if (k > 0 && K[k - 1] == b) return;
  int32_t s = (int32_t)V[k];
  if ((uint32_t)s == b) s = (k + 1 < n && K[k + 1] == b) ? (int32_t)V[k + 1] : -1;
  nxt[b] = s;
}

__global__ void __launch_bounds__(256) k_perm_chase(int64_t k0, int64_t n, const uint32_t *K, const uint32_t *V,
                                                    const int32_t *nxt, const int64_t *ts, int64_t *out) {
  const int64_t k = k0 + (int64_t)blockIdx.x * blockDim.x + threadIdx.x;
  if (k >= n) return;
  const uint32_t b = K[k], p = V[k];
  int64_t q = b;
  if (k + 1 < n && K[k + 1] == b) {
    int32_t c = (int32_t)V[k + 1], d;
    while ((d = nxt[c]) >= 0) c = d;
    q = c;
  }
  out[p] = ts[q];
}

constexpr int PK_UNITS = 512;
__global__ void __launch_bounds__(256) k_perm_keys(int64_t total, const uint32_t *jall, const int64_t *u_off,
                                                   const int64_t *u_n, int32_t n_units, uint32_t *keys,
                                                   int32_t *nxt) {
  __shared__ int64_t s_off[PK_UNITS], s_n[PK_UNITS];
  for (int i = threadIdx.x; i < n_units; i += 256) {
    s_off[i] = u_off[i];
    s_n[i] = u_n[i];
  }
  __syncthreads();
  const int64_t g = (int64_t)blockIdx.x * blockDim.x + threadIdx.x;
  if (g >= total) return;
  int lo = 0, hi = n_units - 1;
  while (lo < hi) {
    const int mid = (lo + hi + 1) >> 1;
    if (s_off[mid] <= g) lo = mid; else hi = mid - 1;
  }
  const int64_t k = g - s_off[lo];
  keys[g] = k < s_n[lo] ? (uint32_t)(s_off[lo] + jall[g]) : (uint32_t)g;
  nxt[g] = -1;
}

__device__ __forceinline__ double mt_double(const uint32_t *w, int64_t k) {
  int32_t a = (int32_t)(w[2 * k] >> 5), b = (int32_t)(w[2 * k + 1] >> 6);
  return (a * 67108864.0 + b) / 9007199254740992.0;
}

struct GeoFlags {
  int64_t *idx;
  uint32_t *count;
  uint32_t cap;
};

__device__ __forceinline__ int64_t geometric_draw(double U, double p, double log_q, GeoFlags fl, int64_t k) {
  if (p >= 0.333333333333333333333333) {
    double sum = p, prod = p, q = 1.0 - p;
    int64_t X = 1;
    while (U > sum) { prod *= q; sum += prod; X++; }
    return X;
  }
  double qv = log1p(-U) / log_q;
  double r = rint(qv);
  if (fabs(qv - r) <= 1e-12 * fmax(1.0, fabs(qv))) {
    uint32_t s = atomicAdd(fl.count, 1u);
    if (s < fl.cap) fl.idx[s] = k;
  }
  return (int64_t)ceil(qv);
}

struct LoadGeo {
  const uint32_t *w; double p, log_q; GeoFlags fl;
  __device__ int64_t operator()(int64_t k) const { return geometric_draw(mt_double(w, k), p, log_q, fl, k); }
};
struct LoadArr {
  const int64_t *a;
  __device__ int64_t operator()(int64_t k) const { return a[k]; }
};
__global__ void k_geo_array(int64_t n, const uint32_t *w, double p, double log_q, GeoFlags fl, int64_t *g) {
  int64_t k = (int64_t)blockIdx.x * blockDim.x + threadIdx.x;
  if (k < n) g[k] = geometric_draw(mt_double(w, k), p, log_q, fl, k);
}
struct StoreTs {
  int64_t *ts; int64_t add; NodeIdx ni;
  __device__ void operator()(int64_t k, int64_t incl, int64_t) const { ts[k] = ts_pack(ni, incl + add); }
};

constexpr int TLEN_PER = 8;
__global__ void __launch_bounds__(256) k_tlen(int64_t n, const uint32_t *w, const double *cum_tlen, int32_t n_tlen,
                                              int64_t rlen, int64_t p_max, const int64_t *ts, int64_t *te,
                                              uint8_t *keep) {
  extern __shared__ __attribute__((aligned(16))) double s_cum[];
  for (int i = threadIdx.x; i < n_tlen; i += blockDim.x) s_cum[i] = cum_tlen[i];
  __syncthreads();
  for (int q = 0; q < TLEN_PER; q++) {
    const int64_t k = ((int64_t)blockIdx.x * TLEN_PER + q) * blockDim.x + threadIdx.x;
    if (k >= n) return;
    const double u = mt_double(w, k);
    int32_t lo = 0, hi = n_tlen;
    while (lo < hi) {
      const int32_t mid = (lo + hi) >> 1;
      if (s_cum[mid] < u) lo = mid + 1; else hi = mid;
    }
    const int64_t tl = lo < rlen ? rlen : lo;
    const int64_t e = (ts[k] & TS_POS_MASK) + tl;
    te[k] = e;
    keep[k] = e < p_max;
  }
}
struct LoadKeep {
  const uint8_t *keep;
  __device__ int64_t operator()(int64_t k) const { return keep[k]; }
};
struct StoreCompact {
  const uint8_t *keep; const int64_t *ts, *te; int64_t *pos0, *pos1; int64_t rlen;
  const uint32_t *wfo; int8_t *fo0;
  int32_t *n0;
  __device__ void operator()(int64_t k, int64_t, int64_t excl) const {
    if (!keep[k]) return;
    const int64_t v = ts[k];
    pos0[excl] = v & TS_POS_MASK;
    if (n0) n0[excl] = (int32_t)(v >> TS_NODE_SHIFT) - 1;
    pos1[excl] = te[k] - rlen;
// ... 112 lines not shown
      if (base + k < count) out[base + k] = w;
    });
    uint32_t *tmp = o; o = nw; nw = tmp;
  }
}

}

int32_t mt_stream_words(mh_ctx *ctx, hipStream_t st, uint32_t seed, int64_t first, int64_t count, DevBuf &out,
                        DevBuf &jobs_buf, int64_t *lead) {
  const int64_t SEG = seg_words();
  const int64_t k0 = first / SEG, k1 = (first + std::max<int64_t>(count, 1) - 1) / SEG;
  *lead = first - k0 * SEG;
  MH_TRY(ensure(ctx, out, 4 * (size_t)((k1 - k0 + 1) * SEG) + 64));
  std::vector<SegJob> jobs;
  for (int64_t k = k0; k <= k1; k++)
    jobs.push_back(SegJob{(uint32_t *)out.p, (k - k0) * SEG, std::min(SEG, first + count - k * SEG), seed, (int32_t)k});
  MH_TRY(ensure_polys(ctx, st, k1, SEG));
  MH_TRY(ensure(ctx, jobs_buf, sizeof(SegJob) * jobs.size() + 64));
  HIPCHK(ctx, hipMemcpyAsync(jobs_buf.p, jobs.data(), sizeof(SegJob) * jobs.size(), hipMemcpyHostToDevice, st));
  hipLaunchKernelGGL(k_mt_segments, dim3((unsigned)jobs.size()), dim3(256), 0, st, (const SegJob *)jobs_buf.p,
                     (const uint32_t *)ctx->jump_polys.p);
  HIPCHK(ctx, hipGetLastError());
  SYNCCHK(ctx, hipStreamSynchronize(st));
  return MH_OK;
}

int32_t mt_state_words(mh_ctx *ctx, hipStream_t st, const uint32_t *key624, int32_t pos, int64_t count, DevBuf &out,
                       DevBuf &key_buf) {
  if (pos < 0 || pos > 624) return arg_fail(ctx, MH_E_ARG, "MT19937 state position outside 0..624");
  MH_TRY(ensure(ctx, out, 4 * (size_t)count + 64));
  MH_TRY(ensure(ctx, key_buf, 4 * 624));
  HIPCHK(ctx, hipMemcpyAsync(key_buf.p, key624, 4 * 624, hipMemcpyHostToDevice, st));
  hipLaunchKernelGGL(k_mt_state, dim3(1), dim3(256), 0, st, (const uint32_t *)key_buf.p, pos, count,
                     (uint32_t *)out.p);
  HIPCHK(ctx, hipGetLastError());
  SYNCCHK(ctx, hipStreamSynchronize(st));
  return MH_OK;
}

namespace {

struct UnitPlan {
  NodeIdx ni;
  int64_t p_min, p_max, n, n_fo_words, n_shuf_words;
  uint32_t s_tloc, s_tlen, s_shuf, s_fo;
  int64_t w_tloc, w_tlen, w_fo, w_shuf;
  int64_t j_off;
  TplSet *out;
};

int32_t decode_parallel(mh_ctx *ctx, const std::vector<DecJob> &dec, int64_t *d_status, bool *done) {
  hipStream_t st = ctx->stream;
  *done = false;
  const int64_t div = 128;
  const int64_t minw = 64;
  std::vector<ChunkJob> cj;
  std::vector<int64_t> s0;
  std::vector<int32_t> first(dec.size() + 1, 0);
  for (size_t u = 0; u < dec.size(); u++) {
    first[u] = (int32_t)cj.size();
    double i = (double)(dec[u].n - 1);
    for (int64_t b = 0; b < dec[u].n_words;) {
      int64_t size = DC_CHUNK;
      while (size > minw && (double)size * (double)div > i) size >>= 1;
      cj.push_back(ChunkJob{dec[u].words, dec[u].n_words, b, dec[u].j, 0, (int32_t)size});
      s0.push_back(b == 0 ? dec[u].n - 1 : (i >= 1.0 ? (int64_t)llround(i) : 0));
      double rem = (double)size;
      while (rem > 0 && i >= 1.0) {
        uint32_t ii = (uint32_t)i, m = ii;
        m |= m >> 1; m |= m >> 2; m |= m >> 4; m |= m >> 8; m |= m >> 16;
        const double rate = (i + 1.0) / ((double)m + 1.0);
        const double lo = (double)((m >> 1) + 1);
        const double need = (i - lo + 1.0) / rate;
        if (need >= rem) { i -= rem * rate; rem = 0; }
        else { i = lo - 1.0; rem -= need; }
      }
      b += size;
    }
  }
  first[dec.size()] = (int32_t)cj.size();
  const int64_t C = (int64_t)cj.size();
  if (C == 0) {
    *done = true;
    return MH_OK;
  }
  const int32_t U = (int32_t)dec.size();
  const int64_t tail_at = (int64_t)1 << 15;
  std::vector<int32_t> tail_c(U, -1);
  for (int32_t u = 0; u < U; u++)
    for (int32_t c = first[u]; c < first[u + 1] && tail_at > 0; c++)
      if (s0[c] < tail_at) {
        tail_c[u] = c;
        for (int32_t k = c; k < first[u + 1]; k++) cj[k].tail = 1;
        break;
      }
  const int32_t tile_sz = DR_TILE;
  std::vector<DecTile> tiles;
  for (int32_t u = 0; u < U; u++) {
    const int32_t ft = (int32_t)tiles.size();
    for (int32_t b = first[u]; b < first[u + 1]; b += tile_sz)
      tiles.push_back(DecTile{u, b, std::min(b + tile_sz, first[u + 1]), ft});
  }
  const int32_t T = (int32_t)tiles.size();
  const size_t bytes = ((sizeof(ChunkJob) * C + 15) / 16) * 16 + 8 * C * 2 + 8 * U * 2 + sizeof(TailJob) * U +
                       sizeof(DecTile) * (T + 1) + 4 * C * 2 + 8 * C + 512;
  MH_TRY(ensure(ctx, ctx->dec_buf, bytes));
  char *p = (char *)ctx->dec_buf.p;
  ChunkJob *d_jobs = (ChunkJob *)p;
  int64_t *d_s0 = (int64_t *)(p + ((sizeof(ChunkJob) * C + 15) / 16) * 16);
  int64_t *d_s1 = d_s0 + C;
  int64_t *d_ndraw = d_s1 + C;
  int64_t *d_rem = d_ndraw + U;
  TailJob *d_tail = (TailJob *)(d_rem + U);
  DecTile *d_tiles = (DecTile *)(d_tail + U);
  int32_t *d_count = (int32_t *)(d_tiles + T + 1);
  int32_t *d_todo = d_count + C;
  int32_t *d_margin = d_todo + C;
  int32_t *d_ntodo = d_margin + 2 * C;
  std::vector<int64_t> ndraw(U);
  for (int32_t u = 0; u < U; u++) ndraw[u] = dec[u].n;
  std::vector<TailJob> tj;
  for (int32_t u = 0; u < U; u++)
    if (tail_c[u] >= 0 && dec[u].n > 0)
      tj.push_back(TailJob{dec[u].words, dec[u].n_words, cj[tail_c[u]].base, d_s1 + tail_c[u], dec[u].j, dec[u].status});
  HIPCHK(ctx, hipMemcpyAsync(d_jobs, cj.data(), sizeof(ChunkJob) * C, hipMemcpyHostToDevice, st));
  HIPCHK(ctx, hipMemcpyAsync(d_s0, s0.data(), 8 * C, hipMemcpyHostToDevice, st));
  HIPCHK(ctx, hipMemcpyAsync(d_tiles, tiles.data(), sizeof(DecTile) * T, hipMemcpyHostToDevice, st));
  HIPCHK(ctx, hipMemcpyAsync(d_ndraw, ndraw.data(), 8 * U, hipMemcpyHostToDevice, st));
  if (!tj.empty()) HIPCHK(ctx, hipMemcpyAsync(d_tail, tj.data(), sizeof(TailJob) * tj.size(), hipMemcpyHostToDevice, st));
  HIPCHK(ctx, hipMemsetAsync(d_ntodo, 0, 8, st));
  const unsigned grid = (unsigned)std::min<int64_t>(C, 4096);
  constexpr int MAX_PASSES = 64;
  const int PASS_BATCH = 24;
  hipLaunchKernelGGL(k_decode_chunks<false>, dim3(grid), dim3(DC_THREADS), 0, st, (const ChunkJob *)d_jobs,
                     (const int32_t *)nullptr, (const int32_t *)nullptr, (int32_t)C, (const int64_t *)d_s0, d_count,
                     d_margin);
  HIPCHK(ctx, hipGetLastError());
  bool conv = false;
  int passes = 1;
  while (passes < MAX_PASSES) {
    int32_t *cur = d_ntodo;
    for (int k = 0; k < PASS_BATCH; k++, passes++) {
      cur = d_ntodo + (passes & 1);
      int32_t *nxt = d_ntodo + ((passes + 1) & 1);
      const unsigned g = passes < 4 ? grid : std::min(grid, 1024u);
      hipLaunchKernelGGL(k_decode_resolve, dim3(T), dim3(DR_THREADS), 0, st, (const DecTile *)d_tiles,
                         (const int64_t *)d_ndraw, (const int32_t *)d_count, (const int32_t *)d_margin, d_s0, d_s1,
                         d_todo, cur, nxt, d_rem);
      hipLaunchKernelGGL(k_decode_chunks<false>, dim3(g), dim3(DC_THREADS), 0, st, (const ChunkJob *)d_jobs,
                         (const int32_t *)d_todo, (const int32_t *)cur, (int32_t)C, (const int64_t *)d_s0, d_count,
                         d_margin);
    }
    HIPCHK(ctx, hipGetLastError());
    int64_t *hs = pinned_small(ctx);
    if (!hs) return arg_fail(ctx, MH_E_OOM, "pinned host memory");
    HIPCHK(ctx, hipMemcpyAsync(hs + 32, cur, 4, hipMemcpyDeviceToHost, st));
    SYNCCHK(ctx, hipStreamSynchronize(st));
    const int32_t h_ntodo = (int32_t)(hs[32] & 0xffffffff);
    if (h_ntodo == 0) {
      conv = true;
      break;
    }
  }
  ctx->dec_passes = passes;
  if (!conv) return MH_OK;
  hipLaunchKernelGGL(k_decode_chunks<true>, dim3(grid), dim3(DC_THREADS), 0, st, (const ChunkJob *)d_jobs,
                     (const int32_t *)nullptr, (const int32_t *)nullptr, (int32_t)C, (const int64_t *)d_s1, d_count,
                     d_margin);
  HIPCHK(ctx, hipGetLastError());
  for (int32_t u = 0; u < U; u++)
    if (dec[u].n > 0 && tail_c[u] < 0) HIPCHK(ctx, hipMemcpyAsync(dec[u].status, d_rem + u, 8, hipMemcpyDeviceToDevice, st));
  if (!tj.empty()) {
    hipLaunchKernelGGL(k_decode_tail, dim3((unsigned)tj.size()), dim3(64), 0, st, (const TailJob *)d_tail);
    HIPCHK(ctx, hipGetLastError());
  }
  for (size_t u = 0; u < dec.size(); u++)
    if (dec[u].n > 0) HIPCHK(ctx, hipMemsetAsync(dec[u].j, 0, 4, st));
  SYNCCHK(ctx, hipStreamSynchronize(st));
  *done = true;
  return MH_OK;
}

template <class KIn>
static hipError_t perm_sort(void *tmp, size_t &tmp_bytes, KIn keys_in, uint32_t *keys_out, uint32_t *vals_out,
                            size_t n, unsigned end_bit, hipStream_t st) {
  return lsd_sort_pairs_iota(tmp, tmp_bytes, keys_in, keys_out, vals_out, (int64_t)n, end_bit, st);
}

struct BatchPerm {
  int64_t *ts, *tsh;
};

int32_t finish_unit(mh_ctx *ctx, UnitPlan &u, const uint32_t *words, const uint32_t *jarr, double p, int32_t rlen,
                    const double *d_cum, int32_t n_tlen, int32_t rng_mode, bool exact, int64_t *d_m,
                    uint32_t *d_flag, int lane = 0, int phase = 0, const BatchPerm *bp = nullptr) {
  hipStream_t st = lane == 0 ? ctx->stream : lane == 1 ? ctx->stream2 : ctx->xstream[lane - 2];
  ctx->stage_stream = lane ? st : nullptr;
  struct Restore {
    mh_ctx *c;
    ~Restore() { c->stage_stream = nullptr; }
  } restore{ctx};
  mh::DevBuf *S4 = lane == 0 ? ctx->s + 4 : lane == 1 ? ctx->lane2 : ctx->xlane[lane - 2];
  mh::DevBuf &perm_tmp = lane == 0 ? ctx->perm_tmp : S4[7];
  void *scan_partials = lane == 0 ? ctx->scan_partials.p : lane == 1 ? ctx->scan_partials2.p : ctx->xscan[lane - 2].p;
  const int64_t n = u.n;
  const uint32_t *w_tloc = words + u.w_tloc, *w_tlen = words + u.w_tlen, *w_fo = words + u.w_fo;
  int64_t *ts = bp ? bp->ts + u.j_off : (int64_t *)S4[0].p;
  int64_t *ts_shuf = (int64_t *)S4[1].p, *te = (int64_t *)S4[2].p;
  uint32_t *sk = (uint32_t *)S4[4].p, *sv = (uint32_t *)S4[5].p;
  int32_t *nxt = (int32_t *)S4[6].p;
  const bool permute = rng_mode == MH_RNG_MITTY && n > 1 && !bp;
  uint8_t *keep = (uint8_t *)S4[3].p;
  int64_t *flag_idx = (int64_t *)ctx->s[11].p;
  int64_t *tot = (int64_t *)((char *)ctx->d_small.p + 128 + 64 * lane);
  const double log_q = std::log(1.0 - p);
  GeoFlags fl{flag_idx, d_flag, 1024};

  if (phase != 2) {
    stage_begin(ctx, "sample_geometric_scan");
    if (!exact) {
      HIPCHK(ctx, device_scan_sum<int64_t>(st, n, LoadGeo{w_tloc, p, log_q, fl}, StoreTs{ts, u.p_min + 1, u.ni},
                                           scan_partials, tot));
    } else {
      int64_t *g = (int64_t *)ctx->s[12].p;
      uint32_t nflag = 0;
      HIPCHK(ctx, hipMemsetAsync(d_flag, 0, 4, st));
      hipLaunchKernelGGL(k_geo_array, dim3(grid_for(n, 256, INT32_MAX)), dim3(256), 0, st, n, w_tloc, p, log_q, fl, g);
      HIPCHK(ctx, hipMemcpyAsync(&nflag, d_flag, 4, hipMemcpyDeviceToHost, st));
      SYNCCHK(ctx, hipStreamSynchronize(st));
      auto host_geo = [&](const uint32_t *ww) {
        double U = (((int32_t)(ww[0] >> 5)) * 67108864.0 + ((int32_t)(ww[1] >> 6))) / 9007199254740992.0;
        return (int64_t)std::ceil(std::log1p(-U) / std::log(1.0 - p));
      };
      if (ctx->force_geo && p < 0.333333333333333333333333) {
        std::vector<uint32_t> hw(2 * (size_t)n);
        std::vector<int64_t> hg((size_t)n);
        HIPCHK(ctx, hipMemcpy(hw.data(), w_tloc, 8 * (size_t)n, hipMemcpyDeviceToHost));
        for (int64_t k = 0; k < n; k++) hg[k] = host_geo(hw.data() + 2 * k);
        HIPCHK(ctx, hipMemcpy(g, hg.data(), 8 * (size_t)n, hipMemcpyHostToDevice));
      } else {
        if (nflag > 1024) return arg_fail(ctx, MH_E_ARG, "too many near-integer geometric quotients");
        std::vector<int64_t> idx(nflag);
        if (nflag) HIPCHK(ctx, hipMemcpy(idx.data(), flag_idx, 8 * nflag, hipMemcpyDeviceToHost));
        for (int64_t k : idx) {
          uint32_t ww[2];
          HIPCHK(ctx, hipMemcpy(ww, w_tloc + 2 * k, 8, hipMemcpyDeviceToHost));
          int64_t gv = host_geo(ww);
          HIPCHK(ctx, hipMemcpy(g + k, &gv, 8, hipMemcpyHostToDevice));
        }
      }
      HIPCHK(ctx, hipMemsetAsync(d_flag, 0, 4, st));
      HIPCHK(ctx, device_scan<int64_t>(st, n, LoadArr{g}, StoreTs{ts, u.p_min + 1, u.ni}, OpSum{}, (int64_t)0,
                                       (int64_t *)scan_partials, tot));
    }
    stage_end(ctx);

    if (permute) {
      stage_begin(ctx, "sample_permutation");
      unsigned end_bit = 1;
      while (end_bit < 32 && ((int64_t)1 << end_bit) < n) end_bit++;
      size_t tmp = 0;
      HIPCHK(ctx, perm_sort(nullptr, tmp, jarr, sk, sv, (size_t)n, end_bit, st));
      MH_TRY(ensure(ctx, perm_tmp, tmp + 256));
      HIPCHK(ctx, perm_sort(perm_tmp.p, tmp, jarr, sk, sv, (size_t)n, end_bit, st));
      HIPCHK(ctx, hipMemsetAsync(nxt, 0xff, 4 * (size_t)n, st));
      hipLaunchKernelGGL(k_perm_heads, dim3(grid_for(n, 256, INT32_MAX)), dim3(256), 0, st, n, (const uint32_t *)sk,
                         (const uint32_t *)sv, nxt);
      HIPCHK(ctx, hipGetLastError());
      stage_end(ctx);
    }
  }
  if (phase == 1) return MH_OK;

  const int64_t *ts_use = bp && rng_mode == MH_RNG_MITTY && n > 1 ? bp->tsh + u.j_off : ts;
  if (permute) {
    stage_begin(ctx, "sample_permutation");
    hipLaunchKernelGGL(k_perm_chase, dim3(grid_for(n, 256, INT32_MAX)), dim3(256), 0, st, (int64_t)0, n,
                       (const uint32_t *)sk, (const uint32_t *)sv, (const int32_t *)nxt, (const int64_t *)ts, ts_shuf);
    HIPCHK(ctx, hipGetLastError());
    stage_end(ctx);
    ts_use = ts_shuf;
  }

  stage_begin(ctx, "sample_tlen_compact");
  hipLaunchKernelGGL(k_tlen, dim3(grid_for((n + TLEN_PER - 1) / TLEN_PER, 256, INT32_MAX)), dim3(256), 8 * n_tlen, st,
                     n, w_tlen, d_cum, n_tlen,
                     (int64_t)rlen, u.p_max, ts_use, te, keep);
  HIPCHK(ctx, hipGetLastError());
  HIPCHK(ctx, device_scan_sum<int64_t>(st, n, LoadKeep{keep},
                                       StoreCompact{keep, ts_use, te, (int64_t *)u.out->pos0.p,
                                                    (int64_t *)u.out->pos1.p, (int64_t)rlen, w_fo,
                                                    (int8_t *)u.out->fo0.p,
                                                    u.out->has_n0 ? (int32_t *)u.out->n0.p : nullptr},
                                       scan_partials, d_m));
  stage_end(ctx);
  return MH_OK;
}

}

struct SampleState {
  std::vector<UnitPlan> plan;
  int32_t n_units = 0, rng_mode = 0, rlen = 0, n_tlen = 0, n_lanes = 1;
  bool two_lanes = false, batch = false;
  double p = 0;
  int64_t j_total = 0, nn = 0;
  uint32_t *words = nullptr, *jall = nullptr;
  double *d_cum = nullptr;
  int64_t *d_m = nullptr, *d_status = nullptr;
  uint32_t *d_flags = nullptr;
  BatchPerm bp{nullptr, nullptr};
  std::vector<hipEvent_t> ev;
  int32_t n_pending = 0;
  ~SampleState() {
    for (hipEvent_t e : ev)
      if (e) (void)hipEventDestroy(e);
  }
};

static void plan_unit_words(UnitPlan &q, int64_t p_min, int64_t p_max, uint64_t seed, double p, int32_t rng_mode,
                            int64_t &words_total) {
  q.p_min = p_min;
  q.p_max = p_max;
  q.n = (int64_t)((double)(q.p_max - q.p_min) * p * 1.2);
  if (q.n < 0) q.n = 0;
  HostMT sr;
  sr.seed((uint32_t)seed);
  q.s_tloc = (uint32_t)sr.interval(0xfffffffeull);
  q.s_tlen = (uint32_t)sr.interval(0xfffffffeull);
  q.s_shuf = (uint32_t)sr.interval(0xfffffffeull);
  q.s_fo = (uint32_t)sr.interval(0xfffffffeull);
  q.n_fo_words = (q.n + 3) / 4 + 1;
  q.n_shuf_words = rng_mode == MH_RNG_MITTY ? shuffle_words_alloc(q.n) : 0;
  auto take = [&](int64_t cnt) {
    int64_t at = words_total;
    words_total = (words_total + cnt + 4 + 3) & ~(int64_t)3;
    return at;
  };
  q.w_tloc = take(2 * q.n);
  q.w_tlen = take(2 * q.n);
  q.w_fo = take(q.n_fo_words);
  q.w_shuf = take(q.n_shuf_words);
}

static void unit_seg_jobs(uint32_t *words, const UnitPlan &q, std::vector<SegJob> &jobs, int64_t &kmax) {
  const int64_t SEG_WORDS = seg_words();
  auto add_stream = [&](uint32_t *out, int64_t count, uint32_t seed) {
    for (int64_t k = 0; k * SEG_WORDS < count; k++) {
      int64_t s0 = k * SEG_WORDS;
      jobs.push_back(SegJob{out, s0, std::min(SEG_WORDS, count - s0), seed, (int32_t)k});
      kmax = std::max(kmax, k);
    }
  };
  add_stream(words + q.w_tloc, 2 * q.n, q.s_tloc);
  add_stream(words + q.w_tlen, 2 * q.n, q.s_tlen);
  add_stream(words + q.w_fo, q.n_fo_words, q.s_fo);
  add_stream(words + q.w_shuf, q.n_shuf_words, q.s_shuf);
}

static int32_t sample_head(mh_ctx *ctx, SampleState &S, int32_t n_units, const int32_t *tpl_ids, const int64_t *p_min,
                           const int64_t *p_max, const uint64_t *seeds, double p, int32_t rlen, const double *cum_tlen,
                           int32_t n_tlen, int32_t rng_mode, const NodeIdx *nidx) {
  for (int32_t u = 0; u < n_units; u++)
    if (seeds[u] > 0xffffffffull)
      return arg_fail(ctx, MH_E_SEED, "Seed value " + std::to_string(seeds[u]) + " is out of range 0 - 4294967295");
  if (n_tlen <= 0 || n_tlen > 8192) return arg_fail(ctx, MH_E_ARG, "cum_tlen must have 1..8192 entries");
  if (rng_mode != MH_RNG_MITTY && rng_mode != MH_RNG_PHILOX) return arg_fail(ctx, MH_E_ARG, "unknown rng_mode");
  MH_TRY(tpl_resolve_all(ctx));
  hipStream_t st = ctx->stream;

  std::vector<UnitPlan> plan(n_units);
  int64_t words_total = 0, j_total = 0, n_max = 1;
  for (int32_t u = 0; u < n_units; u++) {
    UnitPlan &q = plan[u];
    plan_unit_words(q, p_min[u], p_max[u], seeds[u], p, rng_mode, words_total);
    if (q.n > ((int64_t)1 << 30) - 8) return arg_fail(ctx, MH_E_ARG, "region too large for one work unit");
    q.j_off = j_total; j_total += q.n + 4;
    n_max = std::max(n_max, q.n);
    TplSet &ts = ctx->tsets[tpl_ids[u]];
    MH_TRY(wait_unused(ctx, ts.used, ts.used_set));
    MH_TRY(ensure(ctx, ts.fo0, q.n + 16));
    MH_TRY(ensure(ctx, ts.pos0, 8 * (q.n + 16)));
    MH_TRY(ensure(ctx, ts.pos1, 8 * (q.n + 16)));
    q.ni = nidx ? nidx[u] : NodeIdx{};
    ts.n_draws = q.n;
    ts.has_n0 = q.ni.nd != nullptr;
    if (ts.has_n0) MH_TRY(ensure(ctx, ts.n0, 4 * (q.n + 16)));
    ts.valid = false;
    q.out = &ts;
  }
  const int64_t nn = n_max + 1;
  ctx->batch_left = 0;
  for (const UnitPlan &q : plan) ctx->batch_left += q.n;
  PrefetchedWords &pw = ctx->pf_words;
  const bool have_words = rng_mode == MH_RNG_MITTY && pw.valid && pw.p == p && pw.seeds.size() == (size_t)n_units &&
                          std::equal(pw.seeds.begin(), pw.seeds.end(), seeds) &&
                          std::equal(pw.p_min.begin(), pw.p_min.end(), p_min) &&
                          std::equal(pw.p_max.begin(), pw.p_max.end(), p_max) && pw.words_total == words_total;
  pw.valid = false;
  if (have_words) std::swap(ctx->s[0], pw.buf);
  MH_TRY(ensure(ctx, ctx->s[0], 4 * (size_t)words_total + 64));
  MH_TRY(ensure(ctx, ctx->s[3], 4 * (size_t)j_total + 64));
  MH_TRY(ensure(ctx, ctx->s[4], 8 * nn));
  MH_TRY(ensure(ctx, ctx->s[5], 8 * nn));
  MH_TRY(ensure(ctx, ctx->s[6], 8 * nn));
  MH_TRY(ensure(ctx, ctx->s[7], nn));
  MH_TRY(ensure(ctx, ctx->s[8], 4 * (nn + 1)));
  MH_TRY(ensure(ctx, ctx->s[9], 4 * (nn + 1)));
  MH_TRY(ensure(ctx, ctx->s[10], 4 * nn));
  MH_TRY(ensure(ctx, ctx->s[11], 8 * 1024));
  int n_lanes = std::max(1, std::min(2, (int)n_units));
  const bool two_lanes = n_lanes > 1;
  for (int l = 2; l < n_lanes; l++)
    if (!ctx->xstream[l - 2]) {
      int lo = 0, hi = 0;
      (void)hipDeviceGetStreamPriorityRange(&lo, &hi);
      HIPCHK(ctx, hipStreamCreateWithPriority(&ctx->xstream[l - 2], hipStreamNonBlocking, hi));
      HIPCHK(ctx, hipEventCreateWithFlags(&ctx->ev_xjoin[l - 2], hipEventDisableTiming));
    }
  for (int l = 1; l < n_lanes; l++) {
    mh::DevBuf *L = l == 1 ? ctx->lane2 : ctx->xlane[l - 2];
    MH_TRY(ensure(ctx, L[0], 8 * nn));
    MH_TRY(ensure(ctx, L[1], 8 * nn));
    MH_TRY(ensure(ctx, L[2], 8 * nn));
    MH_TRY(ensure(ctx, L[3], nn));
    MH_TRY(ensure(ctx, L[4], 4 * (nn + 1)));
    MH_TRY(ensure(ctx, L[5], 4 * (nn + 1)));
    MH_TRY(ensure(ctx, L[6], 4 * nn));
    MH_TRY(ensure(ctx, l == 1 ? ctx->scan_partials2 : ctx->xscan[l - 2],
                  std::max<size_t>(16 * scan_partials_count(nn + 1) + 64, scan_lb_scratch_bytes<int64_t>(nn + 1))));
  }
  MH_TRY(ensure(ctx, ctx->s[13], 8 * (size_t)n_tlen + 64));
  MH_TRY(ensure(ctx, ctx->s[1], 64 * (size_t)n_units + 64));
  MH_TRY(ensure(ctx, ctx->d_small, 8192 + 256));
  MH_TRY(ensure(ctx, ctx->scan_partials, std::max<size_t>(16 * scan_partials_count(nn + 1) + 64,
                                                           scan_lb_scratch_bytes<int64_t>(nn + 1))));
  uint32_t *words = (uint32_t *)ctx->s[0].p, *jall = (uint32_t *)ctx->s[3].p;
  double *d_cum = (double *)ctx->s[13].p;
  int64_t *d_m = (int64_t *)ctx->s[1].p;
  int64_t *d_status = d_m + n_units;
  uint32_t *d_flags = (uint32_t *)(d_status + n_units);
  HIPCHK(ctx, hipMemsetAsync(ctx->s[1].p, 0, 64 * (size_t)n_units + 64, st));
  HIPCHK(ctx, hipMemcpyAsync(d_cum, cum_tlen, 8 * n_tlen, hipMemcpyHostToDevice, st));

  stage_begin(ctx, "sample");
  if (rng_mode == MH_RNG_MITTY) {
    std::vector<SegJob> jobs;
    std::vector<DecJob> dec;
    int64_t kmax = 0;
    const int64_t SEG_WORDS = seg_words();
    for (int32_t u = 0; u < n_units; u++) {
      UnitPlan &q = plan[u];
      if (q.n == 0) continue;
      unit_seg_jobs(words, q, jobs, kmax);
      dec.push_back(DecJob{words + q.w_shuf, q.n_shuf_words, q.n, jall + q.j_off, d_status + u});
    }
    if (!jobs.empty()) {
      MH_TRY(ensure_polys(ctx, st, kmax, SEG_WORDS));
      MH_TRY(ensure(ctx, ctx->s[2], sizeof(SegJob) * jobs.size() + sizeof(DecJob) * dec.size() + 64));
      SegJob *d_jobs = (SegJob *)ctx->s[2].p;
      DecJob *d_dec = (DecJob *)((char *)ctx->s[2].p + ((sizeof(SegJob) * jobs.size() + 15) / 16) * 16);
      HIPCHK(ctx, hipMemcpyAsync(d_jobs, jobs.data(), sizeof(SegJob) * jobs.size(), hipMemcpyHostToDevice, st));
      HIPCHK(ctx, hipMemcpyAsync(d_dec, dec.data(), sizeof(DecJob) * dec.size(), hipMemcpyHostToDevice, st));
      if (!have_words) {
        stage_begin(ctx, "sample_mt_segments");
        hipLaunchKernelGGL(k_mt_segments, dim3((unsigned)jobs.size()), dim3(256), 0, st, (const SegJob *)d_jobs,
                           (const uint32_t *)ctx->jump_polys.p);
        HIPCHK(ctx, hipGetLastError());
        stage_end(ctx);
      }
      stage_begin(ctx, "sample_shuffle_decode");
      bool done = false;
      if (!ctx->decode_sequential) MH_TRY(decode_parallel(ctx, dec, d_status, &done));
      if (!done) {
        hipLaunchKernelGGL(k_shuffle_decode2, dim3((unsigned)dec.size()), dim3(DC_THREADS), 0, st,
                           (const DecJob *)d_dec);
        HIPCHK(ctx, hipGetLastError());
      }
      stage_end(ctx);
      SYNCCHK(ctx, hipStreamSynchronize(st));
    }
  } else {
    for (int32_t u = 0; u < n_units; u++) {
      UnitPlan &q = plan[u];
      if (q.n == 0) continue;
      uint64_t key = ((uint64_t)q.s_tloc << 32) | q.s_tlen;
      hipLaunchKernelGGL(k_philox_words, dim3(grid_for((2 * q.n + 3) / 4, 256, INT32_MAX)), dim3(256), 0, st,
                         words + q.w_tloc, 2 * q.n, key, 1u);
      hipLaunchKernelGGL(k_philox_words, dim3(grid_for((2 * q.n + 3) / 4, 256, INT32_MAX)), dim3(256), 0, st,
                         words + q.w_tlen, 2 * q.n, key, 2u);
      hipLaunchKernelGGL(k_philox_words, dim3(grid_for((q.n_fo_words + 3) / 4, 256, INT32_MAX)), dim3(256), 0, st,
                         words + q.w_fo, q.n_fo_words, key, 3u);
      HIPCHK(ctx, hipGetLastError());
    }
  }

  if (two_lanes) {
    HIPCHK(ctx, hipEventRecord(ctx->ev_fork, st));
    HIPCHK(ctx, hipStreamWaitEvent(ctx->stream2, ctx->ev_fork, 0));
    for (int l = 2; l < n_lanes; l++) HIPCHK(ctx, hipStreamWaitEvent(ctx->xstream[l - 2], ctx->ev_fork, 0));
  }
  const bool batch = rng_mode == MH_RNG_MITTY && j_total < ((int64_t)1 << 30) && n_units <= PK_UNITS;
  if (batch) {
    MH_TRY(ensure(ctx, ctx->pb[0], 8 * (size_t)j_total + 64));
    MH_TRY(ensure(ctx, ctx->pb[1], 8 * (size_t)j_total + 64));
    for (int b = 2; b < 6; b++) MH_TRY(ensure(ctx, ctx->pb[b], 4 * (size_t)j_total + 64));
    BatchPerm bp{(int64_t *)ctx->pb[0].p, (int64_t *)ctx->pb[1].p};
    for (int32_t u = 0, k = 0; u < n_units; u++) {
      if (plan[u].n == 0) continue;
      MH_TRY(finish_unit(ctx, plan[u], words, jall + plan[u].j_off, p, rlen, d_cum, n_tlen, rng_mode, false, d_m + u,
                         d_flags + u, k++ % n_lanes, 1, &bp));
    }
    if (two_lanes) {
      HIPCHK(ctx, hipEventRecord(ctx->ev_join, ctx->stream2));
      HIPCHK(ctx, hipStreamWaitEvent(st, ctx->ev_join, 0));
      for (int l = 2; l < n_lanes; l++) {
        HIPCHK(ctx, hipEventRecord(ctx->ev_xjoin[l - 2], ctx->xstream[l - 2]));
        HIPCHK(ctx, hipStreamWaitEvent(st, ctx->ev_xjoin[l - 2], 0));
      }
    }
    stage_begin(ctx, "sample_permutation");
    std::vector<int64_t> uo(n_units), un(n_units);
    for (int32_t u = 0; u < n_units; u++) {
      uo[u] = plan[u].j_off;
      un[u] = plan[u].n;
    }
    int64_t *d_uo = (int64_t *)ctx->s[12].p;
    MH_TRY(ensure(ctx, ctx->s[12], 16 * (size_t)n_units + 64));
    d_uo = (int64_t *)ctx->s[12].p;
    HIPCHK(ctx, hipMemcpyAsync(d_uo, uo.data(), 8 * n_units, hipMemcpyHostToDevice, st));
    HIPCHK(ctx, hipMemcpyAsync(d_uo + n_units, un.data(), 8 * n_units, hipMemcpyHostToDevice, st));
    uint32_t *gk = (uint32_t *)ctx->pb[2].p, *sk = (uint32_t *)ctx->pb[3].p, *sv = (uint32_t *)ctx->pb[4].p;
    int32_t *nxt = (int32_t *)ctx->pb[5].p;
    hipLaunchKernelGGL(k_perm_keys, dim3(grid_for(j_total, 256, INT32_MAX)), dim3(256), 0, st, j_total,
                       (const uint32_t *)jall, (const int64_t *)d_uo, (const int64_t *)(d_uo + n_units), n_units, gk,
                       nxt);
    HIPCHK(ctx, hipGetLastError());
    unsigned end_bit = 1;
    while (end_bit < 32 && ((int64_t)1 << end_bit) < j_total) end_bit++;
    size_t tmp = 0;
    HIPCHK(ctx, perm_sort(nullptr, tmp, gk, sk, sv, (size_t)j_total, end_bit, st));
    MH_TRY(ensure(ctx, ctx->pb_tmp, tmp + 256));
    HIPCHK(ctx, perm_sort(ctx->pb_tmp.p, tmp, gk, sk, sv, (size_t)j_total, end_bit, st));
    hipLaunchKernelGGL(k_perm_heads, dim3(grid_for(j_total, 256, INT32_MAX)), dim3(256), 0, st, j_total,
                       (const uint32_t *)sk, (const uint32_t *)sv, nxt);
    HIPCHK(ctx, hipGetLastError());
    stage_end(ctx);
    S.bp = bp;
  } else {
    for (int32_t u = 0, k = 0; u < n_units; u++) {
      if (plan[u].n == 0) continue;
      MH_TRY(finish_unit(ctx, plan[u], words, jall + plan[u].j_off, p, rlen, d_cum, n_tlen, rng_mode, false, d_m + u,
                         d_flags + u, k++ % n_lanes));
    }
  }
  S.plan = std::move(plan);
  S.n_units = n_units;
  S.rng_mode = rng_mode;
  S.rlen = rlen;
  S.n_tlen = n_tlen;
  S.n_lanes = n_lanes;
  S.two_lanes = two_lanes;
  S.batch = batch;
  S.p = p;
  S.j_total = j_total;
  S.nn = nn;
  S.words = words;
  S.jall = jall;
  S.d_cum = d_cum;
  S.d_m = d_m;
  S.d_status = d_status;
  S.d_flags = d_flags;
  return MH_OK;
}

static int32_t sample_tail(mh_ctx *ctx, SampleState &S, int64_t *out_n) {
  hipStream_t st = ctx->stream;
  std::vector<UnitPlan> &plan = S.plan;
  const int32_t n_units = S.n_units, rng_mode = S.rng_mode, rlen = S.rlen, n_tlen = S.n_tlen, n_lanes = S.n_lanes;
  const bool two_lanes = S.two_lanes;
  const double p = S.p;
  const int64_t j_total = S.j_total, nn = S.nn;
  uint32_t *words = S.words, *jall = S.jall;
  double *d_cum = S.d_cum;
  int64_t *d_m = S.d_m, *d_status = S.d_status;
  uint32_t *d_flags = S.d_flags;
  if (S.batch) {
    const BatchPerm &bp = S.bp;
    const uint32_t *sk = (const uint32_t *)ctx->pb[3].p, *sv = (const uint32_t *)ctx->pb[4].p;
    const int32_t *nxt = (const int32_t *)ctx->pb[5].p;
    stage_begin(ctx, "sample_permutation");
    hipLaunchKernelGGL(k_perm_chase, dim3(grid_for(j_total, 256, INT32_MAX)), dim3(256), 0, st, (int64_t)0, j_total,
                       sk, sv, nxt, (const int64_t *)bp.ts, bp.tsh);
    HIPCHK(ctx, hipGetLastError());
    stage_end(ctx);
    if (two_lanes) {
      HIPCHK(ctx, hipEventRecord(ctx->ev_fork, st));
      HIPCHK(ctx, hipStreamWaitEvent(ctx->stream2, ctx->ev_fork, 0));
      for (int l = 2; l < n_lanes; l++) HIPCHK(ctx, hipStreamWaitEvent(ctx->xstream[l - 2], ctx->ev_fork, 0));
    }
    for (int32_t u = 0, k = 0; u < n_units; u++) {
      if (plan[u].n == 0) continue;
      MH_TRY(finish_unit(ctx, plan[u], words, jall + plan[u].j_off, p, rlen, d_cum, n_tlen, rng_mode, false, d_m + u,
                         d_flags + u, k++ % n_lanes, 2, &bp));
    }
  }
  if (two_lanes) {
    HIPCHK(ctx, hipEventRecord(ctx->ev_join, ctx->stream2));
    HIPCHK(ctx, hipStreamWaitEvent(st, ctx->ev_join, 0));
    for (int l = 2; l < n_lanes; l++) {
      HIPCHK(ctx, hipEventRecord(ctx->ev_xjoin[l - 2], ctx->xstream[l - 2]));
      HIPCHK(ctx, hipStreamWaitEvent(st, ctx->ev_xjoin[l - 2], 0));
    }
  }
  std::vector<int64_t> hm(n_units), hstat(n_units);
  std::vector<uint32_t> hflag(n_units);
  int64_t *hs = pinned_small(ctx);
  const size_t rb_bytes = 20 * (size_t)n_units;
  if (hs && rb_bytes <= 3072) {
    HIPCHK(ctx, hipMemcpyAsync(hs + 64, d_m, rb_bytes, hipMemcpyDeviceToHost, st));
    SYNCCHK(ctx, hipStreamSynchronize(st));
    std::memcpy(hm.data(), hs + 64, 8 * n_units);
    std::memcpy(hstat.data(), hs + 64 + n_units, 8 * n_units);
    std::memcpy(hflag.data(), hs + 64 + 2 * n_units, 4 * n_units);
  } else {
    HIPCHK(ctx, hipMemcpyAsync(hm.data(), d_m, 8 * n_units, hipMemcpyDeviceToHost, st));
    HIPCHK(ctx, hipMemcpyAsync(hstat.data(), d_status, 8 * n_units, hipMemcpyDeviceToHost, st));
    HIPCHK(ctx, hipMemcpyAsync(hflag.data(), d_flags, 4 * n_units, hipMemcpyDeviceToHost, st));
    SYNCCHK(ctx, hipStreamSynchronize(st));
  }

  for (int32_t u = 0; u < n_units; u++) {
    UnitPlan &q = plan[u];
    if (q.n == 0) continue;
    if (ctx->force_fixup) hstat[u] = 1;
    if (ctx->force_geo) hflag[u] = 1;
    if (hstat[u] == 0 && hflag[u] == 0) continue;
    if (rng_mode == MH_RNG_MITTY && hstat[u] != 0) {
      hipLaunchKernelGGL(k_shuffle_decode, dim3(1), dim3(SD_THREADS), 0, st, q.s_shuf, q.n, jall + q.j_off);
      HIPCHK(ctx, hipGetLastError());
    }
    MH_TRY(ensure(ctx, ctx->s[12], 8 * (size_t)nn));
    HIPCHK(ctx, hipMemsetAsync(d_flags + u, 0, 4, st));
    MH_TRY(finish_unit(ctx, q, words, jall + q.j_off, p, rlen, d_cum, n_tlen, rng_mode, hflag[u] != 0, d_m + u,
                       d_flags + u));
    HIPCHK(ctx, hipMemcpyAsync(&hm[u], d_m + u, 8, hipMemcpyDeviceToHost, st));
    SYNCCHK(ctx, hipStreamSynchronize(st));
    ctx->fixups++;
  }
  stage_end(ctx);
  for (int32_t u = 0; u < n_units; u++) {
    TplSet &ts = *plan[u].out;
    ts.n = plan[u].n == 0 ? 0 : hm[u];
    ts.rlen = rlen;
    ts.valid = true;
    if (out_n) out_n[u] = ts.n;
  }
  return MH_OK;
}

__global__ void k_unit_result(const int64_t *m, const int64_t *status, const uint32_t *flag, int64_t *out) {
  if (threadIdx.x == 0) {
    out[0] = *m;
    out[1] = *status;
    out[2] = (int64_t)*flag;
  }
}

static int32_t sample_tail_async(mh_ctx *ctx, const std::shared_ptr<SampleState> &Sp) {
  SampleState &S = *Sp;
  std::vector<UnitPlan> &plan = S.plan;
  const int32_t n_units = S.n_units;
  hipStream_t st = ctx->stream, l1 = ctx->stream2;
  const BatchPerm &bp = S.bp;
  const uint32_t *sk = (const uint32_t *)ctx->pb[3].p, *sv = (const uint32_t *)ctx->pb[4].p;
  const int32_t *nxt = (const int32_t *)ctx->pb[5].p;
  HIPCHK(ctx, hipEventRecord(ctx->ev_fork, st));
  HIPCHK(ctx, hipStreamWaitEvent(l1, ctx->ev_fork, 0));
  S.ev.assign(n_units, nullptr);
  for (int32_t u = 0; u < n_units; u++) {
    UnitPlan &q = plan[u];
    TplSet &ts = *q.out;
    if (q.n == 0) {
      ts.n = 0;
      ts.rlen = S.rlen;
      ts.valid = true;
      continue;
    }
    ctx->stage_stream = l1;
    stage_begin(ctx, "sample_permutation");
    const int64_t k0 = q.j_off, k1 = q.j_off + q.n + 4;
    hipLaunchKernelGGL(k_perm_chase, dim3(grid_for(k1 - k0, 256, INT32_MAX)), dim3(256), 0, l1, k0, k1, sk, sv, nxt,
                       (const int64_t *)bp.ts, bp.tsh);
    stage_end(ctx);
    ctx->stage_stream = nullptr;
    HIPCHK(ctx, hipGetLastError());
    MH_TRY(finish_unit(ctx, q, S.words, S.jall + q.j_off, S.p, S.rlen, S.d_cum, S.n_tlen, S.rng_mode, false,
                       S.d_m + u, S.d_flags + u, 1, 2, &bp));
    hipLaunchKernelGGL(k_unit_result, dim3(1), dim3(64), 0, l1, (const int64_t *)(S.d_m + u),
                       (const int64_t *)(S.d_status + u), (const uint32_t *)(S.d_flags + u), ctx->d_units + 4 * u);
    HIPCHK(ctx, hipGetLastError());
    HIPCHK(ctx, hipEventCreateWithFlags(&S.ev[u], hipEventDisableTiming));
    HIPCHK(ctx, hipEventRecord(S.ev[u], l1));
    ts.pend = u;
    S.n_pending++;
  }
  stage_end(ctx);
  if (S.n_pending) ctx->tail_state = Sp;
  return MH_OK;
}

int32_t tpl_resolve(mh_ctx *ctx, TplSet &ts) {
  if (ts.pend < 0) return MH_OK;
  const int32_t u = ts.pend;
  ts.pend = -1;
  auto Sp = std::static_pointer_cast<SampleState>(ctx->tail_state);
  if (!Sp || u >= Sp->n_units || Sp->plan[u].out != &ts)
    return arg_fail(ctx, MH_E_STATE, "template set of a lost sampling batch");
  SampleState &S = *Sp;
  UnitPlan &q = S.plan[u];
  hipStream_t st = ctx->stream;
  SYNCCHK(ctx, hipEventSynchronize(S.ev[u]));
  const volatile int64_t *r = ctx->h_units + 4 * u;
  int64_t m = r[0];
  const int64_t status = ctx->force_fixup ? 1 : r[1];
  const uint32_t flag = ctx->force_geo ? 1u : (uint32_t)r[2];
  HIPCHK(ctx, hipStreamWaitEvent(st, S.ev[u], 0));
  if (status != 0 || flag != 0) {
    if (S.rng_mode == MH_RNG_MITTY && status != 0) {
      hipLaunchKernelGGL(k_shuffle_decode, dim3(1), dim3(SD_THREADS), 0, st, q.s_shuf, q.n, S.jall + q.j_off);
      HIPCHK(ctx, hipGetLastError());
    }
    MH_TRY(ensure(ctx, ctx->s[12], 8 * (size_t)S.nn));
    HIPCHK(ctx, hipMemsetAsync(S.d_flags + u, 0, 4, st));
    MH_TRY(finish_unit(ctx, q, S.words, S.jall + q.j_off, S.p, S.rlen, S.d_cum, S.n_tlen, S.rng_mode, flag != 0,
                       S.d_m + u, S.d_flags + u));
    HIPCHK(ctx, hipMemcpyAsync(&m, S.d_m + u, 8, hipMemcpyDeviceToHost, st));
    SYNCCHK(ctx, hipStreamSynchronize(st));
    ctx->fixups++;
  }
  ts.n = m;
  ts.rlen = S.rlen;
  ts.valid = true;
  if (--S.n_pending == 0) ctx->tail_state.reset();
  return MH_OK;
}

int32_t tpl_resolve_all(mh_ctx *ctx) {
  auto Sp = std::static_pointer_cast<SampleState>(ctx->tail_state);
  if (!Sp) return MH_OK;
  for (UnitPlan &q : Sp->plan)
    if (q.out && q.out->pend >= 0) MH_TRY(tpl_resolve(ctx, *q.out));
  return MH_OK;
}

int32_t prefetch_words(mh_ctx *ctx, hipStream_t st, int32_t n_units, const int64_t *p_min, const int64_t *p_max,
                       const uint64_t *seeds, double p) {
  PrefetchedWords &pw = ctx->pf_words;
  pw.valid = false;
  std::vector<UnitPlan> plan(n_units);
  int64_t words_total = 0;
  for (int32_t u = 0; u < n_units; u++) {
    plan_unit_words(plan[u], p_min[u], p_max[u], seeds[u], p, MH_RNG_MITTY, words_total);
    if (plan[u].n > ((int64_t)1 << 30) - 8) return MH_OK;
  }
  MH_TRY(ensure(ctx, pw.buf, 4 * (size_t)words_total + 64));
  std::vector<SegJob> jobs;
  int64_t kmax = 0;
  for (const UnitPlan &q : plan)
    if (q.n > 0) unit_seg_jobs((uint32_t *)pw.buf.p, q, jobs, kmax);
// ... 45 lines not shown
```

### mitty_amd/csrc/mh_sort.h

```cpp
#pragma once

#include <hip/hip_runtime.h>

#include <cstdint>

#include "mh_device.h"
#include "mh_scan.h"

namespace mh {

constexpr int RS_THREADS = 512;
constexpr int RS_ITEMS = 16;
constexpr int RS_TILE = RS_THREADS * RS_ITEMS;
constexpr int RS_WAVES = RS_THREADS / 64;
constexpr int RS_BITS = 9;
constexpr uint32_t RS_BINS = 1u << RS_BITS, RS_MASK = RS_BINS - 1u;
constexpr int RS_DPT = (int)RS_BINS / RS_THREADS;
static_assert(RS_DPT >= 1 && RS_DPT * RS_THREADS == (int)RS_BINS, "every thread owns whole digits");
constexpr int RS_MAXP = 4;
constexpr uint32_t RS_AGG = 0x40000000u, RS_INC = 0x80000000u, RS_VAL = 0x3fffffffu;

static __global__ void __launch_bounds__(RS_THREADS) k_rs_hist(const uint32_t *keys, int64_t n, int passes,
                                                              uint32_t *ghist) {
  __shared__ uint32_t h[RS_MAXP * RS_BINS];
  for (int i = threadIdx.x; i < RS_MAXP * (int)RS_BINS; i += RS_THREADS) h[i] = 0;
  __syncthreads();
  for (int64_t i = (int64_t)blockIdx.x * RS_THREADS + threadIdx.x; i < n; i += (int64_t)gridDim.x * RS_THREADS) {
    const uint32_t k = keys[i];
    for (int p = 0; p < passes; p++) atomicAdd(&h[p * RS_BINS + ((k >> (RS_BITS * p)) & RS_MASK)], 1u);
  }
  __syncthreads();
  for (int i = threadIdx.x; i < passes * (int)RS_BINS; i += RS_THREADS)
    if (h[i]) atomicAdd(&ghist[i], h[i]);
}

static __global__ void __launch_bounds__(RS_THREADS) k_rs_starts(uint32_t *ghist) {
  __shared__ int32_t wsum[RS_WAVES];
  uint32_t *h = ghist + (size_t)blockIdx.x * RS_BINS;
  const int tid = threadIdx.x, lane = tid & 63, w = tid >> 6;
  uint32_t v[RS_DPT], s = 0;
#pragma unroll
  for (int q = 0; q < RS_DPT; q++) {
    v[q] = h[RS_DPT * tid + q];
    s += v[q];
  }
  int total;
  const int32_t incl = wave_sum_incl((int32_t)s, total);
  if (lane == 63) wsum[w] = incl;
  __syncthreads();
  int32_t pre = 0;
#pragma unroll
  for (int q = 0; q < RS_WAVES; q++) pre += q < w ? wsum[q] : 0;
  uint32_t x = (uint32_t)(pre + incl) - s;
#pragma unroll
  for (int q = 0; q < RS_DPT; q++) {
    h[RS_DPT * tid + q] = x;
    x += v[q];
  }
}

static __global__ void __launch_bounds__(RS_THREADS) k_rs_onesweep(const uint32_t *keys_in, const uint32_t *vals_in,
                                                                  int64_t n, int shift, const uint32_t *gstart,
                                                                  uint32_t *status, uint32_t *keys_out, uint32_t *vals_out,
                                                                  uint32_t *fault) {
  __shared__ uint32_t wc[RS_WAVES][RS_BINS];
  __shared__ uint32_t ds[RS_BINS];
  __shared__ uint32_t go[RS_BINS];
  __shared__ uint32_t sb[RS_TILE];
  __shared__ int32_t wsum[RS_WAVES];
  __shared__ uint32_t s_tile;
  const int tid = threadIdx.x, lane = tid & 63, w = tid >> 6;
  uint32_t *ticket = status;
  uint32_t *st = status + 16;
  if (tid == 0) s_tile = atomicAdd(ticket, 1u);
  for (int i = tid; i < RS_WAVES * (int)RS_BINS; i += RS_THREADS) (&wc[0][0])[i] = 0;
  __syncthreads();
  const int64_t tile = s_tile;
  const int64_t t0 = tile * RS_TILE;
  const int nt = (int)(n - t0 < RS_TILE ? n - t0 : RS_TILE);
  const int wb = w * (64 * RS_ITEMS) + lane;
  const uint64_t below = lane ? (~0ull >> (64 - lane)) : 0ull;
  uint32_t key[RS_ITEMS], rk[RS_ITEMS];
#pragma unroll
  for (int k = 0; k < RS_ITEMS; k++)
    key[k] = wb + 64 * k < nt ? keys_in[t0 + wb + 64 * k] : 0xffffffffu;
#pragma unroll
  for (int k = 0; k < RS_ITEMS; k++) {
    const bool ok = wb + 64 * k < nt;
    const uint32_t d = (key[k] >> shift) & RS_MASK;
    uint64_t m = __ballot(ok);
#pragma unroll
    for (int b = 0; b < RS_BITS; b++) {
      const uint64_t bal = __ballot(ok && ((d >> b) & 1u));
      m &= ((d >> b) & 1u) ? bal : ~bal;
    }
    const int leader = m ? __builtin_ctzll(m) : lane;
    uint32_t c0 = 0;
    if (ok && lane == leader) c0 = wc[w][d];
    c0 = __shfl(c0, leader, 64);
    rk[k] = c0 + (uint32_t)__popcll(m & below);
    if (ok && lane == leader) wc[w][d] = c0 + (uint32_t)__popcll(m);
  }
  __syncthreads();
  uint32_t t[RS_DPT], s = 0;
#pragma unroll
  for (int q = 0; q < RS_DPT; q++) {
    const int d = RS_DPT * tid + q;
    uint32_t c = 0;
#pragma unroll
    for (int x = 0; x < RS_WAVES; x++) {
      const uint32_t y = wc[x][d];
      wc[x][d] = c;
      c += y;
    }
    t[q] = c;
    s += c;
    __hip_atomic_store(&st[tile * RS_BINS + d], (tile == 0 ? RS_INC : RS_AGG) | c, __ATOMIC_RELAXED,
                       __HIP_MEMORY_SCOPE_AGENT);
  }
  {
    int total;
    const int32_t incl = wave_sum_incl((int32_t)s, total);
    if (lane == 63) wsum[w] = incl;
    __syncthreads();
    int32_t pre = 0;
#pragma unroll
    for (int q = 0; q < RS_WAVES; q++) pre += q < w ? wsum[q] : 0;
    uint32_t x = (uint32_t)(pre + incl) - s;
#pragma unroll
    for (int q = 0; q < RS_DPT; q++) {
      ds[RS_DPT * tid + q] = x;
      x += t[q];
    }
  }
#pragma unroll
  for (int q = 0; q < RS_DPT; q++) {
    const int d = RS_DPT * tid + q;
    uint32_t pre = 0;
    if (tile > 0) {
      int64_t j = tile - 1;
      uint32_t spins = 0;
      for (;;) {
        const uint32_t v = __hip_atomic_load(&st[j * RS_BINS + d], __ATOMIC_RELAXED, __HIP_MEMORY_SCOPE_AGENT);
        if (v & (RS_INC | RS_AGG)) {
          pre += v & RS_VAL;
          if (v & RS_INC) break;
          j--;
          continue;
        }
        if (++spins > (1u << 24)) {
          if (fault) __hip_atomic_store(fault, 1u, __ATOMIC_RELAXED, __HIP_MEMORY_SCOPE_SYSTEM);
          break;
        }
        __builtin_amdgcn_s_sleep(1);
      }
      __hip_atomic_store(&st[tile * RS_BINS + d], RS_INC | (pre + t[q]), __ATOMIC_RELAXED, __HIP_MEMORY_SCOPE_AGENT);
    }
    go[d] = gstart[d] + pre;
  }
  __syncthreads();
#pragma unroll
  for (int k = 0; k < RS_ITEMS; k++) {
    if (wb + 64 * k < nt) {
      const uint32_t d = (key[k] >> shift) & RS_MASK;
      rk[k] = ds[d] + wc[w][d] + rk[k];
      sb[rk[k]] = key[k];
    }
  }
  __syncthreads();
  uint32_t oi[RS_ITEMS];
#pragma unroll
  for (int k = 0; k < RS_ITEMS; k++) {
    const int p = k * RS_THREADS + tid;
    oi[k] = 0xffffffffu;
    if (p < nt) {
      const uint32_t kk = sb[p], d = (kk >> shift) & RS_MASK;
      const uint32_t o = go[d] + (uint32_t)p - ds[d];
      if ((int64_t)o < n) {
        keys_out[o] = kk;
        oi[k] = o;
      }
    }
  }
  __syncthreads();
#pragma unroll
  for (int k = 0; k < RS_ITEMS; k++) {
    const int li = wb + 64 * k;
    if (li < nt) sb[rk[k]] = vals_in ? vals_in[t0 + li] : (uint32_t)(t0 + li);
  }
  __syncthreads();
#pragma unroll
  for (int k = 0; k < RS_ITEMS; k++)
    if (oi[k] != 0xffffffffu) vals_out[oi[k]] = sb[k * RS_THREADS + tid];
}

inline size_t lsd_sort_tmp_bytes(int64_t n) {
  const int64_t tiles = (n + RS_TILE - 1) / RS_TILE;
  return 2 * 4 * (size_t)n + 4 * (size_t)(tiles < 1 ? 1 : tiles) * RS_BINS + 64 + 4 * RS_MAXP * RS_BINS + 2048;
}

inline hipError_t lsd_sort_pairs_iota(void *tmp, size_t &tmp_bytes, const uint32_t *keys_in, uint32_t *keys_out,
                                      uint32_t *vals_out, int64_t n, unsigned end_bit, hipStream_t st) {
  if (!tmp) {
    tmp_bytes = lsd_sort_tmp_bytes(n);
    return hipSuccess;
  }
  if (tmp_bytes < lsd_sort_tmp_bytes(n) || n < 0 || n >= ((int64_t)1 << 30)) return hipErrorInvalidValue;
  if (n == 0) return hipSuccess;
  const int64_t tiles = (n + RS_TILE - 1) / RS_TILE;
  char *p = (char *)tmp;
  auto take = [&](size_t b) {
    char *q = p;
    p += (b + 255) & ~(size_t)255;
    return q;
  };
  uint32_t *k2 = (uint32_t *)take(4 * (size_t)n), *v2 = (uint32_t *)take(4 * (size_t)n);
  const size_t st_bytes = 64 + 4 * (size_t)tiles * RS_BINS;
  uint32_t *status = (uint32_t *)take(st_bytes);
  uint32_t *ghist = (uint32_t *)take(4 * RS_MAXP * RS_BINS);
  const int passes = end_bit == 0 ? 1 : (int)((end_bit + RS_BITS - 1) / RS_BITS);
  hipError_t e = hipMemsetAsync(ghist, 0, 4 * (size_t)passes * RS_BINS, st);
  if (e != hipSuccess) return e;
  const int64_t hg = tiles < 2048 ? tiles : 2048;
  hipLaunchKernelGGL(k_rs_hist, dim3((unsigned)hg), dim3(RS_THREADS), 0, st, keys_in, n, passes, ghist);
  hipLaunchKernelGGL(k_rs_starts, dim3((unsigned)passes), dim3(RS_THREADS), 0, st, ghist);
  if ((e = hipGetLastError()) != hipSuccess) return e;
  const uint32_t *ksrc = keys_in, *vsrc = nullptr;
  for (int ps = 0; ps < passes; ps++) {
    const bool to_out = ((passes - 1 - ps) & 1) == 0;
    uint32_t *kd = to_out ? keys_out : k2, *vd = to_out ? vals_out : v2;
    if ((e = hipMemsetAsync(status, 0, st_bytes, st)) != hipSuccess) return e;
    hipLaunchKernelGGL(k_rs_onesweep, dim3((unsigned)tiles), dim3(RS_THREADS), 0, st, ksrc, vsrc, n, RS_BITS * ps,
                       (const uint32_t *)(ghist + (size_t)ps * RS_BINS), status, kd, vd, scan_fault_device());
    if ((e = hipGetLastError()) != hipSuccess) return e;
    ksrc = kd;
    vsrc = vd;
  }
  return hipSuccess;
}

}
```

Baseline: 1.723 billion.

## Split permutation sort into unit groups and overlap with scans and emission

Splits the batched permutation radix sort over all draws into up to three contiguous unit groups, each sorted with group-local keys (fewer radix bits) and a base offset re-added in the last pass. The first group is sorted up front and the later groups are deferred into the per-unit chase loop on the second stream, gated by events. Per-unit scans are forked to stream2 before shuffle decode, and a redundant host sync is skipped when decode has already synchronised. The intent is to shorten the critical path by overlapping sort work with other stages, at the cost of more kernel launches and extra event and stream coordination.

```diff
diff --git a/include/mitty_hip.h b/include/mitty_hip.h
--- a/include/mitty_hip.h
+++ b/include/mitty_hip.h
@@ -35,6 +35,8 @@
                          int64_t *incl, int64_t *excl, int64_t *total, int64_t *info);
 int32_t mh_selftest_sort(mh_ctx *ctx, const uint32_t *keys, int64_t n, int32_t end_bit, uint32_t *keys_out,
                          uint32_t *vals_out);
+int32_t mh_selftest_sort_base(mh_ctx *ctx, const uint32_t *keys, int64_t n, int32_t end_bit, uint32_t base,
+                              uint32_t *keys_out, uint32_t *vals_out);
 
 int32_t mh_read_model_params(int64_t mean_rlen, double coverage, double *p, int64_t *passes);
 int32_t mh_work_units(uint64_t seed, const int32_t *ploidy, int64_t n_regions, int64_t passes,
@@ -253,6 +255,8 @@
 #define MH_DEC_FORCE_FIXUP 2
 #define MH_DEC_FORCE_GEO 4
 int32_t mh_set_decode_mode(mh_ctx *ctx, int32_t mode);
+int32_t mh_set_sort_groups(mh_ctx *ctx, int32_t k);
+int32_t mh_sort_group_plan(const int64_t *draws, int32_t n_units, int32_t k, int32_t *bounds, int32_t *n_groups);
 int32_t mh_fixup_count(mh_ctx *ctx, int64_t *n);
 
 #ifdef __cplusplus
diff --git a/mitty_amd/_native.py b/mitty_amd/_native.py
--- a/mitty_amd/_native.py
+++ b/mitty_amd/_native.py
@@ -12,12 +12,12 @@
 MH_RNG_MITTY, MH_RNG_PHILOX = 0, 1
 
 EXPORTS = ['mh_version', 'mh_device_count', 'mh_create', 'mh_destroy', 'mh_last_error', 'mh_sync',
-           'mh_selftest_scan_fault', 'mh_selftest_scan', 'mh_selftest_sort', 'mh_selftest_bgzf',
+           'mh_selftest_scan_fault', 'mh_selftest_scan', 'mh_selftest_sort', 'mh_selftest_sort_base', 'mh_selftest_bgzf',
            'mh_read_model_params', 'mh_work_units', 'mh_upload_contig', 'mh_release_contig', 'mh_build_haplotype', 'mh_upload_variants', 'mh_build_haplotype_vset', 'mh_build_haplotypes_vset', 'mh_prefetch_haplotypes_vset', 'mh_release_variants', 'mh_get_nodes', 'mh_get_haplotype_aux',
            'mh_release_haplotype', 'mh_expand_variant', 'mh_sample_templates', 'mh_sample_templates_span', 'mh_set_templates',
            'mh_get_templates', 'mh_templates_export', 'mh_templates_import', 'mh_gc_thin', 'mh_emit_reads', 'mh_emit_prepare', 'mh_emit_reads_async', 'mh_emit_collect', 'mh_output_size', 'mh_output_fetch', 'mh_output_reset', 'mh_host_alloc', 'mh_host_free', 'mh_device_cache_trim', 'mh_device_live_bytes',
            'mh_read_batch', 'mh_set_corruption', 'mh_set_corruption_stream', 'mh_get_corruption_stream', 'mh_stage_times', 'mh_enable_timing', 'mh_sample_units', 'mh_sample_units_async', 'mh_templates_count',
-           'mh_use_templates', 'mh_release_templates', 'mh_mt_window_at', 'mh_fixup_count', 'mh_set_emit_mode', 'mh_set_decode_mode',
+           'mh_use_templates', 'mh_release_templates', 'mh_mt_window_at', 'mh_fixup_count', 'mh_set_emit_mode', 'mh_set_decode_mode', 'mh_set_sort_groups', 'mh_sort_group_plan',
            'mh_emit_reads_range', 'mh_emit_measure', 'mh_count_kept', 'mh_bam_set_refs', 'mh_bam_add_fastq', 'mh_bam_add_output',
            'mh_bam_records', 'mh_bam_set_capacity', 'mh_bam_set_spill_dir', 'mh_bam_spilled', 'mh_bam_export', 'mh_bam_import', 'mh_bam_sort', 'mh_bam_write', 'mh_bam_write_gpu', 'mh_bam_reset', 'mh_bam_partition', 'mh_bam_partition_fetch', 'mh_bam_import_tie', 'mh_bam_sorted_head', 'mh_bam_write_part', 'mh_bam_bai_runs', 'mh_corrupt_fastq', 'mh_bgzf_compress', 'mh_bgzf_eof', 'mh_bgzf_compress_device', 'mh_bgzf_compress_gpu', 'mh_output_bgzf',
            'mh_output_bgzf_range', 'mh_output_bgzf_pair', 'mh_output_bgzf_wait', 'mh_output_fetch_async',
@@ -77,6 +77,7 @@
   _sig(L, 'mh_selftest_scan_fault', [c_vp])
   _sig(L, 'mh_selftest_scan', [c_vp, c_i32, c_i32, c_vp, c_i64, c_i32, c_vp, c_vp, c_vp, c_vp])
   _sig(L, 'mh_selftest_sort', [c_vp, c_vp, c_i64, c_i32, c_vp, c_vp])
+  _sig(L, 'mh_selftest_sort_base', [c_vp, c_vp, c_i64, c_i32, ctypes.c_uint32, c_vp, c_vp])
   _sig(L, 'mh_selftest_bgzf', [c_vp, c_vp, c_i64, c_i32, c_vp, c_i64, P_i64])
   _sig(L, 'mh_read_model_params', [c_i64, c_dbl, ctypes.POINTER(c_dbl), P_i64])
   _sig(L, 'mh_work_units', [c_u64, c_vp, c_i64, c_i64, c_vp, c_vp, c_vp, P_i64])
@@ -208,6 +209,8 @@
   _sig(L, 'mh_fixup_count', [c_vp, P_i64])
   _sig(L, 'mh_set_emit_mode', [c_vp, c_i32])
   _sig(L, 'mh_set_decode_mode', [c_vp, c_i32])
+  _sig(L, 'mh_set_sort_groups', [c_vp, c_i32])
+  _sig(L, 'mh_sort_group_plan', [c_vp, c_i32, c_i32, c_vp, ctypes.POINTER(c_i32)])
   _lib = L
   return L
 
@@ -668,6 +671,9 @@
   def set_decode_mode(self, mode):
     self._chk(self._L.mh_set_decode_mode(self._h, int(mode)))
 
+  def set_sort_groups(self, k):
+    self._chk(self._L.mh_set_sort_groups(self._h, int(k)))
+
   def fixup_count(self):
     n = c_i64()
     self._chk(self._L.mh_fixup_count(self._h, ctypes.byref(n)))
@@ -1189,6 +1195,13 @@
   def sync(self):
     self._chk(self._L.mh_sync(self._h))
 
+  def selftest_sort_base(self, keys, end_bit, base):
+    k = np.ascontiguousarray(keys, dtype=np.uint32)
+    ko, vo = np.empty(max(k.size, 1), np.uint32), np.empty(max(k.size, 1), np.uint32)
+    self._chk(self._L.mh_selftest_sort_base(self._h, k.ctypes.data, k.size, int(end_bit), int(base), ko.ctypes.data,
+                                            vo.ctypes.data))
+    return ko[:k.size], vo[:k.size]
+
   def selftest_sort(self, keys, end_bit):
     import numpy as np
     k = np.ascontiguousarray(keys, dtype=np.uint32)
@@ -1234,3 +1247,13 @@
     _raise(rc, 'mh_expand_variant: bad variant (op {!r}, oplen {})'.format(op, oplen))
   return [(out[5 * j], out[5 * j + 1], chr(out[5 * j + 2]), out[5 * j + 3], out[5 * j + 4])
           for j in range(n.value)], sn.value, rn.value
+
+
+def sort_group_plan(draws, k=-1):
+  d = np.ascontiguousarray(draws, dtype=np.int64)
+  b = np.zeros(4, np.int32)
+  g = c_i32()
+  rc = lib().mh_sort_group_plan(d.ctypes.data, len(d), int(k), b.ctypes.data, ctypes.byref(g))
+  if rc != MH_OK:
+    raise ValueError('mh_sort_group_plan: bad arguments ({})'.format(rc))
+  return [int(x) for x in b[:g.value + 1]]
diff --git a/mitty_amd/csrc/mh_api.hip b/mitty_amd/csrc/mh_api.hip
--- a/mitty_amd/csrc/mh_api.hip
+++ b/mitty_amd/csrc/mh_api.hip
@@ -528,6 +528,8 @@
   cov_release(ctx->cov);
   if (ctx->ev_fork) (void)hipEventDestroy(ctx->ev_fork);
   if (ctx->ev_join) (void)hipEventDestroy(ctx->ev_join);
+  for (hipEvent_t e : ctx->ev_sortg)
+    if (e) (void)hipEventDestroy(e);
   if (ctx->stream2) (void)hipStreamDestroy(ctx->stream2);
   if (ctx->ev_prefetch) (void)hipEventDestroy(ctx->ev_prefetch);
   if (ctx->pstream) (void)hipStreamDestroy(ctx->pstream);
@@ -563,6 +565,11 @@
 
 int32_t mh_selftest_sort(mh_ctx *ctx, const uint32_t *keys, int64_t n, int32_t end_bit, uint32_t *keys_out,
                          uint32_t *vals_out) {
+  return mh_selftest_sort_base(ctx, keys, n, end_bit, 0, keys_out, vals_out);
+}
+
+int32_t mh_selftest_sort_base(mh_ctx *ctx, const uint32_t *keys, int64_t n, int32_t end_bit, uint32_t base,
+                              uint32_t *keys_out, uint32_t *vals_out) {
   CTX_GUARD(ctx);
   if (n < 0 || (n > 0 && (!keys || !keys_out || !vals_out)) || end_bit < 0 || end_bit > 32)
     return arg_fail(ctx, MH_E_ARG, "bad sort arguments");
@@ -575,7 +582,7 @@
   uint32_t *dk = (uint32_t *)b.p, *ko = (uint32_t *)((char *)b.p + kb), *vo = (uint32_t *)((char *)b.p + 2 * kb);
   const int32_t rc = [&]() -> int32_t {
     if (n) HIPCHK(ctx, hipMemcpyAsync(dk, keys, 4 * (size_t)n, hipMemcpyHostToDevice, st));
-    HIPCHK(ctx, lsd_sort_pairs_iota((char *)b.p + 3 * kb, tmp, dk, ko, vo, n, (unsigned)end_bit, st));
+    HIPCHK(ctx, lsd_sort_pairs_iota((char *)b.p + 3 * kb, tmp, dk, ko, vo, n, (unsigned)end_bit, st, base));
     if (n) {
       HIPCHK(ctx, hipMemcpyAsync(keys_out, ko, 4 * (size_t)n, hipMemcpyDeviceToHost, st));
       HIPCHK(ctx, hipMemcpyAsync(vals_out, vo, 4 * (size_t)n, hipMemcpyDeviceToHost, st));
@@ -1606,6 +1613,20 @@
   ctx->decode_sequential = (mode & MH_DEC_SEQUENTIAL) != 0;
   ctx->force_fixup = (mode & MH_DEC_FORCE_FIXUP) != 0;
   ctx->force_geo = (mode & MH_DEC_FORCE_GEO) != 0;
+  return MH_OK;
+}
+
+int32_t mh_set_sort_groups(mh_ctx *ctx, int32_t k) {
+  if (!ctx || k < -1) return MH_E_ARG;
+  ctx->sort_groups = k;
+  return MH_OK;
+}
+
+int32_t mh_sort_group_plan(const int64_t *draws, int32_t n_units, int32_t k, int32_t *bounds, int32_t *n_groups) {
+  if (n_units < 0 || (n_units > 0 && !draws) || k < -1 || !bounds || !n_groups) return MH_E_ARG;
+  for (int32_t u = 0; u < n_units; u++)
+    if (draws[u] < 0 || draws[u] > ((int64_t)1 << 30)) return MH_E_ARG;
+  *n_groups = mh::sort_group_plan(draws, n_units, k, bounds);
   return MH_OK;
 }
 
diff --git a/mitty_amd/csrc/mh_internal.h b/mitty_amd/csrc/mh_internal.h
--- a/mitty_amd/csrc/mh_internal.h
+++ b/mitty_amd/csrc/mh_internal.h
@@ -285,6 +285,9 @@
   mh::DevBuf perm_tmp;
   mh::DevBuf pb[6];
   mh::DevBuf pb_tmp;
+  static constexpr int SORT_GROUPS_MAX = 3;
+  hipEvent_t ev_sortg[SORT_GROUPS_MAX] = {nullptr, nullptr, nullptr};
+  int32_t sort_groups = 0;
   mh::DevBuf gz_slots, gz_info, gz_off, gz_scan, gz_out, gz_in;
   mh::DevBuf gz_tok;
   hipEvent_t ev_gz[2] = {nullptr, nullptr};
@@ -454,6 +457,7 @@
                            int32_t n_tlen, int32_t rng_mode, const NodeIdx *nidx = nullptr);
 int32_t tpl_resolve(mh_ctx *ctx, TplSet &ts);
 int32_t tpl_resolve_all(mh_ctx *ctx);
+int32_t sort_group_plan(const int64_t *draws, int32_t n_units, int32_t k, int32_t *bounds);
 
 int32_t sync_writers(mh_ctx *ctx);
 int32_t bgzf_device(mh_ctx *ctx, hipStream_t st, const uint8_t *d_in, int64_t n, uint8_t *d_out, int64_t cap,
diff --git a/mitty_amd/csrc/mh_sample.hip b/mitty_amd/csrc/mh_sample.hip
--- a/mitty_amd/csrc/mh_sample.hip
+++ b/mitty_amd/csrc/mh_sample.hip
@@ -691,16 +691,16 @@
 }
 
 constexpr int PK_UNITS = 512;
-__global__ void __launch_bounds__(256) k_perm_keys(int64_t total, const uint32_t *jall, const int64_t *u_off,
-                                                   const int64_t *u_n, int32_t n_units, uint32_t *keys,
-                                                   int32_t *nxt) {
+__global__ void __launch_bounds__(256) k_perm_keys(int64_t g0, int64_t total, const uint32_t *jall,
+                                                   const int64_t *u_off, const int64_t *u_n, int32_t n_units,
+                                                   uint32_t *keys, int32_t *nxt) {
   __shared__ int64_t s_off[PK_UNITS], s_n[PK_UNITS];
   for (int i = threadIdx.x; i < n_units; i += 256) {
     s_off[i] = u_off[i];
     s_n[i] = u_n[i];
   }
   __syncthreads();
-  const int64_t g = (int64_t)blockIdx.x * blockDim.x + threadIdx.x;
+  const int64_t g = g0 + (int64_t)blockIdx.x * blockDim.x + threadIdx.x;
   if (g >= total) return;
   int lo = 0, hi = n_units - 1;
   while (lo < hi) {
@@ -708,7 +708,7 @@
     if (s_off[mid] <= g) lo = mid; else hi = mid - 1;
   }
   const int64_t k = g - s_off[lo];
-  keys[g] = k < s_n[lo] ? (uint32_t)(s_off[lo] + jall[g]) : (uint32_t)g;
+  keys[g] = (uint32_t)((k < s_n[lo] ? s_off[lo] + jall[g] : g) - g0);
   nxt[g] = -1;
 }
 
@@ -987,6 +987,7 @@
   first[dec.size()] = (int32_t)cj.size();
   const int64_t C = (int64_t)cj.size();
   if (C == 0) {
+    SYNCCHK(ctx, hipStreamSynchronize(st));
     *done = true;
     return MH_OK;
   }
@@ -1089,8 +1090,8 @@
 
 template <class KIn>
 static hipError_t perm_sort(void *tmp, size_t &tmp_bytes, KIn keys_in, uint32_t *keys_out, uint32_t *vals_out,
-                            size_t n, unsigned end_bit, hipStream_t st) {
-  return lsd_sort_pairs_iota(tmp, tmp_bytes, keys_in, keys_out, vals_out, (int64_t)n, end_bit, st);
+                            size_t n, unsigned end_bit, hipStream_t st, uint32_t base = 0) {
+  return lsd_sort_pairs_iota(tmp, tmp_bytes, keys_in, keys_out, vals_out, (int64_t)n, end_bit, st, base);
 }
 
 struct BatchPerm {
@@ -1216,6 +1217,9 @@
   int64_t *d_m = nullptr, *d_status = nullptr;
   uint32_t *d_flags = nullptr;
   BatchPerm bp{nullptr, nullptr};
+  int32_t n_groups = 0, gb[mh_ctx::SORT_GROUPS_MAX + 1] = {0};
+  int64_t goff[mh_ctx::SORT_GROUPS_MAX + 1] = {0};
+  int64_t *d_uo = nullptr;
   std::vector<hipEvent_t> ev;
   int32_t n_pending = 0;
   ~SampleState() {
@@ -1262,6 +1266,48 @@
   add_stream(words + q.w_tlen, 2 * q.n, q.s_tlen);
   add_stream(words + q.w_fo, q.n_fo_words, q.s_fo);
   add_stream(words + q.w_shuf, q.n_shuf_words, q.s_shuf);
+}
+
+int32_t sort_group_plan(const int64_t *draws, int32_t n_units, int32_t k, int32_t *bounds) {
+  bounds[0] = 0;
+  if (n_units <= 0) return 0;
+  int32_t G = 0;
+  if (k != 0 && n_units >= 2) {
+    int64_t total = 0;
+    for (int32_t u = 0; u < n_units; u++) total += draws[u];
+    auto lead = [&](int64_t num, int64_t den, int32_t lo) {
+      int32_t u = 0;
+      for (int64_t acc = 0; u < n_units - 1 && (acc += draws[u]) * den <= total * num; u++) {}
+      return std::min(std::max(u, lo), n_units - 1);
+    };
+    const int32_t first = k > 0 ? std::min(k, n_units - 1) : lead(1, 8, 1);
+    bounds[++G] = first;
+    if (k < 0 && first + 1 < n_units) bounds[++G] = lead(1, 2, first + 1);
+  }
+  bounds[++G] = n_units;
+  return G;
+}
+
+static int32_t sort_group(mh_ctx *ctx, const SampleState &S, int32_t g, hipStream_t st) {
+  StageStreamScope on_st(ctx, st == ctx->stream ? nullptr : st);
+  StageScope stage(ctx, "sample_permutation");
+  const int64_t o0 = S.goff[g], o1 = S.goff[g + 1], span = o1 - o0;
+  uint32_t *gk = (uint32_t *)ctx->pb[2].p, *sk = (uint32_t *)ctx->pb[3].p, *sv = (uint32_t *)ctx->pb[4].p;
+  int32_t *nxt = (int32_t *)ctx->pb[5].p;
+  hipLaunchKernelGGL(k_perm_keys, dim3(grid_for(span, 256, INT32_MAX)), dim3(256), 0, st, o0, o1,
+                     (const uint32_t *)S.jall, (const int64_t *)S.d_uo, (const int64_t *)(S.d_uo + S.n_units),
+                     S.n_units, gk, nxt);
+  HIPCHK(ctx, hipGetLastError());
+  unsigned end_bit = 1;
+  while (end_bit < 32 && ((int64_t)1 << end_bit) < span) end_bit++;
+  size_t tmp = ctx->pb_tmp.cap;
+  HIPCHK(ctx, perm_sort(ctx->pb_tmp.p, tmp, gk + o0, sk + o0, sv + o0, (size_t)span, end_bit, st, (uint32_t)o0));
+  hipLaunchKernelGGL(k_perm_heads, dim3(grid_for(span, 256, INT32_MAX)), dim3(256), 0, st, span,
+                     (const uint32_t *)(sk + o0), (const uint32_t *)(sv + o0), nxt);
+  HIPCHK(ctx, hipGetLastError());
+  stage.end();
+  HIPCHK(ctx, hipEventRecord(ctx->ev_sortg[g], st));
+  return MH_OK;
 }
 
 static int32_t sample_head(mh_ctx *ctx, SampleState &S, int32_t n_units, const int32_t *tpl_ids, const int64_t *p_min,
@@ -1341,6 +1387,26 @@
   MH_TRY(ensure(ctx, ctx->d_small, 8192 + 256));
   MH_TRY(ensure(ctx, ctx->scan_partials, std::max<size_t>(16 * scan_partials_count(nn + 1) + 64,
                                                            scan_lb_scratch_bytes<int64_t>(nn + 1))));
+  const bool batch = rng_mode == MH_RNG_MITTY && j_total < ((int64_t)1 << 30) && n_units <= PK_UNITS;
+  int32_t gb[mh_ctx::SORT_GROUPS_MAX + 1] = {0};
+  int32_t n_groups = 0;
+  auto group_off = [&](int32_t g) { return g == n_groups ? j_total : plan[gb[g]].j_off; };
+  if (batch) {
+    MH_TRY(ensure(ctx, ctx->pb[0], 8 * (size_t)j_total + 64));
+    MH_TRY(ensure(ctx, ctx->pb[1], 8 * (size_t)j_total + 64));
+    for (int b = 2; b < 6; b++) MH_TRY(ensure(ctx, ctx->pb[b], 4 * (size_t)j_total + 64));
+    std::vector<int64_t> draws(n_units);
+    for (int32_t u = 0; u < n_units; u++) draws[u] = plan[u].n;
+    n_groups = sort_group_plan(draws.data(), n_units, ctx->sort_groups, gb);
+    int64_t span_max = 0;
+    for (int32_t g = 0; g < n_groups; g++) {
+      span_max = std::max(span_max, group_off(g + 1) - group_off(g));
+      if (!ctx->ev_sortg[g]) HIPCHK(ctx, hipEventCreateWithFlags(&ctx->ev_sortg[g], hipEventDisableTiming));
+    }
+    MH_TRY(ensure(ctx, ctx->pb_tmp, lsd_sort_tmp_bytes(span_max) + 256));
+  }
+  const bool scans_early = batch && two_lanes;
+  bool scans_forked = false;
   uint32_t *words = (uint32_t *)ctx->s[0].p, *jall = (uint32_t *)ctx->s[3].p;
   double *d_cum = (double *)ctx->s[13].p;
   int64_t *d_m = (int64_t *)ctx->s[1].p;
@@ -1350,6 +1416,18 @@
   HIPCHK(ctx, hipMemcpyAsync(d_cum, cum_tlen, 8 * n_tlen, hipMemcpyHostToDevice, st));
 
   stage_begin(ctx, "sample");
+  BatchPerm bp{(int64_t *)ctx->pb[0].p, (int64_t *)ctx->pb[1].p};
+  auto fork_scans = [&]() -> int32_t {
+    HIPCHK(ctx, hipEventRecord(ctx->ev_fork, st));
+    HIPCHK(ctx, hipStreamWaitEvent(ctx->stream2, ctx->ev_fork, 0));
+    for (int32_t u = 0; u < n_units; u++) {
+      if (plan[u].n == 0) continue;
+      MH_TRY(finish_unit(ctx, plan[u], words, jall + plan[u].j_off, p, rlen, d_cum, n_tlen, rng_mode, false, d_m + u,
+                         d_flags + u, 1, 1, &bp));
+    }
+    HIPCHK(ctx, hipEventRecord(ctx->ev_join, ctx->stream2));
+    return MH_OK;
+  };
   if (rng_mode == MH_RNG_MITTY) {
     std::vector<SegJob> jobs;
     std::vector<DecJob> dec;
@@ -1375,6 +1453,10 @@
         HIPCHK(ctx, hipGetLastError());
         stage_end(ctx);
       }
+      if (scans_early) {
+        MH_TRY(fork_scans());
+        scans_forked = true;
+      }
       stage_begin(ctx, "sample_shuffle_decode");
       bool done = false;
       if (!ctx->decode_sequential) MH_TRY(decode_parallel(ctx, dec, d_status, &done));
@@ -1384,7 +1466,7 @@
         HIPCHK(ctx, hipGetLastError());
       }
       stage_end(ctx);
-      SYNCCHK(ctx, hipStreamSynchronize(st));
+      if (!done) SYNCCHK(ctx, hipStreamSynchronize(st));
     }
   } else {
     for (int32_t u = 0; u < n_units; u++) {
@@ -1401,59 +1483,38 @@
     }
   }
 
-  if (two_lanes) {
-    HIPCHK(ctx, hipEventRecord(ctx->ev_fork, st));
-    HIPCHK(ctx, hipStreamWaitEvent(ctx->stream2, ctx->ev_fork, 0));
-    for (int l = 2; l < n_lanes; l++) HIPCHK(ctx, hipStreamWaitEvent(ctx->xstream[l - 2], ctx->ev_fork, 0));
-  }
-  const bool batch = rng_mode == MH_RNG_MITTY && j_total < ((int64_t)1 << 30) && n_units <= PK_UNITS;
   if (batch) {
-    MH_TRY(ensure(ctx, ctx->pb[0], 8 * (size_t)j_total + 64));
-    MH_TRY(ensure(ctx, ctx->pb[1], 8 * (size_t)j_total + 64));
-    for (int b = 2; b < 6; b++) MH_TRY(ensure(ctx, ctx->pb[b], 4 * (size_t)j_total + 64));
-    BatchPerm bp{(int64_t *)ctx->pb[0].p, (int64_t *)ctx->pb[1].p};
-    for (int32_t u = 0, k = 0; u < n_units; u++) {
-      if (plan[u].n == 0) continue;
-      MH_TRY(finish_unit(ctx, plan[u], words, jall + plan[u].j_off, p, rlen, d_cum, n_tlen, rng_mode, false, d_m + u,
-                         d_flags + u, k++ % n_lanes, 1, &bp));
-    }
-    if (two_lanes) {
-      HIPCHK(ctx, hipEventRecord(ctx->ev_join, ctx->stream2));
-      HIPCHK(ctx, hipStreamWaitEvent(st, ctx->ev_join, 0));
-      for (int l = 2; l < n_lanes; l++) {
-        HIPCHK(ctx, hipEventRecord(ctx->ev_xjoin[l - 2], ctx->xstream[l - 2]));
-        HIPCHK(ctx, hipStreamWaitEvent(st, ctx->ev_xjoin[l - 2], 0));
-      }
-    }
-    stage_begin(ctx, "sample_permutation");
+    if (!scans_forked)
+      for (int32_t u = 0; u < n_units; u++) {
+        if (plan[u].n == 0) continue;
+        MH_TRY(finish_unit(ctx, plan[u], words, jall + plan[u].j_off, p, rlen, d_cum, n_tlen, rng_mode, false, d_m + u,
+                           d_flags + u, 0, 1, &bp));
+      }
     std::vector<int64_t> uo(n_units), un(n_units);
     for (int32_t u = 0; u < n_units; u++) {
       uo[u] = plan[u].j_off;
       un[u] = plan[u].n;
     }
-    int64_t *d_uo = (int64_t *)ctx->s[12].p;
-    MH_TRY(ensure(ctx, ctx->s[12], 16 * (size_t)n_units + 64));
-    d_uo = (int64_t *)ctx->s[12].p;
+    int64_t *d_uo = (int64_t *)((char *)ctx->s[1].p + 24 * (size_t)n_units);
     HIPCHK(ctx, hipMemcpyAsync(d_uo, uo.data(), 8 * n_units, hipMemcpyHostToDevice, st));
     HIPCHK(ctx, hipMemcpyAsync(d_uo + n_units, un.data(), 8 * n_units, hipMemcpyHostToDevice, st));
-    uint32_t *gk = (uint32_t *)ctx->pb[2].p, *sk = (uint32_t *)ctx->pb[3].p, *sv = (uint32_t *)ctx->pb[4].p;
-    int32_t *nxt = (int32_t *)ctx->pb[5].p;
-    hipLaunchKernelGGL(k_perm_keys, dim3(grid_for(j_total, 256, INT32_MAX)), dim3(256), 0, st, j_total,
-                       (const uint32_t *)jall, (const int64_t *)d_uo, (const int64_t *)(d_uo + n_units), n_units, gk,
-                       nxt);
-    HIPCHK(ctx, hipGetLastError());
-    unsigned end_bit = 1;
-    while (end_bit < 32 && ((int64_t)1 << end_bit) < j_total) end_bit++;
-    size_t tmp = 0;
-    HIPCHK(ctx, perm_sort(nullptr, tmp, gk, sk, sv, (size_t)j_total, end_bit, st));
-    MH_TRY(ensure(ctx, ctx->pb_tmp, tmp + 256));
-    HIPCHK(ctx, perm_sort(ctx->pb_tmp.p, tmp, gk, sk, sv, (size_t)j_total, end_bit, st));
-    hipLaunchKernelGGL(k_perm_heads, dim3(grid_for(j_total, 256, INT32_MAX)), dim3(256), 0, st, j_total,
-                       (const uint32_t *)sk, (const uint32_t *)sv, nxt);
-    HIPCHK(ctx, hipGetLastError());
-    stage_end(ctx);
+    S.n_units = n_units;
+    S.jall = jall;
+    S.d_uo = d_uo;
+    S.n_groups = n_groups;
+    for (int32_t g = 0; g <= n_groups; g++) {
+      S.gb[g] = gb[g];
+      S.goff[g] = group_off(g);
+    }
+    if (n_groups) MH_TRY(sort_group(ctx, S, 0, st));
+    if (scans_forked) HIPCHK(ctx, hipStreamWaitEvent(st, ctx->ev_join, 0));
     S.bp = bp;
   } else {
+    if (two_lanes) {
+      HIPCHK(ctx, hipEventRecord(ctx->ev_fork, st));
+      HIPCHK(ctx, hipStreamWaitEvent(ctx->stream2, ctx->ev_fork, 0));
+      for (int l = 2; l < n_lanes; l++) HIPCHK(ctx, hipStreamWaitEvent(ctx->xstream[l - 2], ctx->ev_fork, 0));
+    }
     for (int32_t u = 0, k = 0; u < n_units; u++) {
       if (plan[u].n == 0) continue;
       MH_TRY(finish_unit(ctx, plan[u], words, jall + plan[u].j_off, p, rlen, d_cum, n_tlen, rng_mode, false, d_m + u,
@@ -1495,6 +1556,7 @@
     const BatchPerm &bp = S.bp;
     const uint32_t *sk = (const uint32_t *)ctx->pb[3].p, *sv = (const uint32_t *)ctx->pb[4].p;
     const int32_t *nxt = (const int32_t *)ctx->pb[5].p;
+    for (int32_t g = 1; g < S.n_groups; g++) MH_TRY(sort_group(ctx, S, g, st));
     stage_begin(ctx, "sample_permutation");
     hipLaunchKernelGGL(k_perm_chase, dim3(grid_for(j_total, 256, INT32_MAX)), dim3(256), 0, st, (int64_t)0, j_total,
                        sk, sv, nxt, (const int64_t *)bp.ts, bp.tsh);
@@ -1577,14 +1639,12 @@
   SampleState &S = *Sp;
   std::vector<UnitPlan> &plan = S.plan;
   const int32_t n_units = S.n_units;
-  hipStream_t st = ctx->stream, l1 = ctx->stream2;
+  hipStream_t l1 = ctx->stream2;
   const BatchPerm &bp = S.bp;
   const uint32_t *sk = (const uint32_t *)ctx->pb[3].p, *sv = (const uint32_t *)ctx->pb[4].p;
   const int32_t *nxt = (const int32_t *)ctx->pb[5].p;
-  HIPCHK(ctx, hipEventRecord(ctx->ev_fork, st));
-  HIPCHK(ctx, hipStreamWaitEvent(l1, ctx->ev_fork, 0));
   S.ev.assign(n_units, nullptr);
-  for (int32_t u = 0; u < n_units; u++) {
+  for (int32_t u = 0, g = 0; u < n_units; u++) {
     UnitPlan &q = plan[u];
     TplSet &ts = *q.out;
     if (q.n == 0) {
@@ -1592,6 +1652,10 @@
       ts.rlen = S.rlen;
       ts.valid = true;
       continue;
+    }
+    for (; g < S.n_groups && S.gb[g] <= u; g++) {
+      if (g == 0) HIPCHK(ctx, hipStreamWaitEvent(l1, ctx->ev_sortg[0], 0));
+      else if (u < S.gb[g + 1]) MH_TRY(sort_group(ctx, S, g, l1));
     }
     ctx->stage_stream = l1;
     stage_begin(ctx, "sample_permutation");
diff --git a/mitty_amd/csrc/mh_sort.h b/mitty_amd/csrc/mh_sort.h
--- a/mitty_amd/csrc/mh_sort.h
+++ b/mitty_amd/csrc/mh_sort.h
@@ -62,7 +62,7 @@
 static __global__ void __launch_bounds__(RS_THREADS) k_rs_onesweep(const uint32_t *keys_in, const uint32_t *vals_in,
                                                                   int64_t n, int shift, const uint32_t *gstart,
                                                                   uint32_t *status, uint32_t *keys_out, uint32_t *vals_out,
-                                                                  uint32_t *fault) {
+                                                                  uint32_t *fault, uint32_t key_base, uint32_t val_base) {
   __shared__ uint32_t wc[RS_WAVES][RS_BINS];
   __shared__ uint32_t ds[RS_BINS];
   __shared__ uint32_t go[RS_BINS];
@@ -177,7 +177,7 @@
       const uint32_t kk = sb[p], d = (kk >> shift) & RS_MASK;
       const uint32_t o = go[d] + (uint32_t)p - ds[d];
       if ((int64_t)o < n) {
-        keys_out[o] = kk;
+        keys_out[o] = kk + key_base;
         oi[k] = o;
       }
     }
@@ -186,7 +186,7 @@
 #pragma unroll
   for (int k = 0; k < RS_ITEMS; k++) {
     const int li = wb + 64 * k;
-    if (li < nt) sb[rk[k]] = vals_in ? vals_in[t0 + li] : (uint32_t)(t0 + li);
+    if (li < nt) sb[rk[k]] = vals_in ? vals_in[t0 + li] : (uint32_t)(t0 + li) + val_base;
   }
   __syncthreads();
 #pragma unroll
@@ -200,7 +200,8 @@
 }
 
 inline hipError_t lsd_sort_pairs_iota(void *tmp, size_t &tmp_bytes, const uint32_t *keys_in, uint32_t *keys_out,
-                                      uint32_t *vals_out, int64_t n, unsigned end_bit, hipStream_t st) {
+                                      uint32_t *vals_out, int64_t n, unsigned end_bit, hipStream_t st,
+                                      uint32_t base = 0) {
   if (!tmp) {
     tmp_bytes = lsd_sort_tmp_bytes(n);
     return hipSuccess;
@@ -231,7 +232,8 @@
     uint32_t *kd = to_out ? keys_out : k2, *vd = to_out ? vals_out : v2;
     if ((e = hipMemsetAsync(status, 0, st_bytes, st)) != hipSuccess) return e;
     hipLaunchKernelGGL(k_rs_onesweep, dim3((unsigned)tiles), dim3(RS_THREADS), 0, st, ksrc, vsrc, n, RS_BITS * ps,
-                       (const uint32_t *)(ghist + (size_t)ps * RS_BINS), status, kd, vd, scan_fault_device());
+                       (const uint32_t *)(ghist + (size_t)ps * RS_BINS), status, kd, vd, scan_fault_device(),
+                       ps == passes - 1 ? base : 0u, base);
     if ((e = hipGetLastError()) != hipSuccess) return e;
     ksrc = kd;
     vsrc = vd;
```

Result: no change. 1.722 billion, median of 3 (-0.0%).
